# PetoAdam/RayZen

Measured on AMD Instinct MI355X. Metric: Msamples/s (rays x spp / s) at 1080p, higher is better.
Workload: dtype f32; 1 GPU; configs[1]: bunny stand-in (bunny69312, 69324 tris incl. floor) 1920x1080, 64 spp per frame (64 spp-equivalents of work per GPU), 4 bounces, 2 lights; width=1920, height=1080, spp_per_gpu=64, spp_total=64, bounces=4, triangles=69324, floor=cube scaled (8, 0.5, 8) at y = -3 (main.cpp:378), parallelism=tiles8x8-roundrobin-x1

## Files before the change

### include/rayzen_hip.h

```cpp
#ifndef RAYZEN_HIP_H
#define RAYZEN_HIP_H

#include <stddef.h>
#include <stdint.h>

#ifdef __cplusplus
extern "C" {
#endif


typedef struct rz_triangle {
    float v0[3]; float pad0;
    float v1[3]; float pad1;
    float v2[3]; float pad2;
    int32_t materialIndex;
    int32_t tail_pad[3];
} rz_triangle;

typedef struct rz_bvh_node {
    float boundsMin[3]; int32_t leftFirst;
    float boundsMax[3]; int32_t count;
} rz_bvh_node;

typedef struct rz_bvh_instance {
// ... 152 lines not shown
int rz_rebuild_geometry(rz_ctx* ctx, double max_ratio, rz_mesh_quality* out, size_t cap, size_t* n_meshes, unsigned flags );

int rz_read_binding(rz_ctx* ctx, rz_binding binding, void* out, size_t bytes, size_t* needed);

int rz_set_frame(rz_ctx* ctx, const rz_frame_params* params);

int rz_set_stream(rz_ctx* ctx, void* hip_stream);
int rz_bind_accum(rz_ctx* ctx, void* device_rgba, size_t bytes);

int rz_render(rz_ctx* ctx);
int rz_render_counted(rz_ctx* ctx, rz_counters* out);
int rz_sync(rz_ctx* ctx);

int rz_clear_accum(rz_ctx* ctx);

int rz_read_accum(rz_ctx* ctx, float* rgba, size_t bytes);

int rz_resolve_rgba8(rz_ctx* ctx, uint8_t* rgba8, size_t bytes);

typedef struct rz_present_params {
    float   fps;
    int32_t show_fps;
    int32_t show_lights;
    int32_t show_bvh;
    int32_t bvh_mode;
    int32_t selected_blas;
    int32_t selected_tri;
} rz_present_params;
int rz_present(rz_ctx* ctx, const rz_present_params* params, uint8_t* rgba8, size_t rgba8_bytes, float* rgb32f,
               size_t rgb32f_bytes);

int rz_last_render_ms(rz_ctx* ctx, float* ms, int* launches);
int rz_render_history_ms(rz_ctx* ctx, float* ms, int cap);
const char* rz_last_kernel_name(const rz_ctx* ctx);

void* rz_accum_device_ptr(rz_ctx* ctx);

int rz_debug_fail_alloc(rz_ctx* ctx, int nth);

void* rz_stream_handle(rz_ctx* ctx);

typedef struct rz_group rz_group;
#define RZ_GROUP_ID_BYTES 128
#define RZ_GROUP_LOOPBACK 0x10000u
int       rz_group_rccl_version(int* version);
int       rz_group_unique_id(void* id128);
rz_group* rz_group_create(int ndev, const int* devices, unsigned flags);
rz_group* rz_group_create_rank(int device, int rank, int nranks, const void* id128, unsigned flags);
void      rz_group_destroy(rz_group* g);
const char* rz_group_last_error(const rz_group* g);
int       rz_group_size(const rz_group* g);
const char* rz_group_transport(const rz_group* g);
int       rz_group_set_transport(rz_group* g, const char* name);
int       rz_group_local_count(const rz_group* g);
int       rz_group_rank(const rz_group* g, int local);
rz_ctx*   rz_group_ctx(rz_group* g, int local);
int rz_group_upload(rz_group* g, rz_binding binding, const void* data, size_t bytes);
int rz_group_update(rz_group* g, rz_binding binding, size_t offset, const void* data, size_t bytes);
int rz_group_set_frame(rz_group* g, const rz_frame_params* params);
int rz_group_render(rz_group* g);
int rz_group_reduce(rz_group* g, int root);
int rz_group_sync(rz_group* g);
int rz_group_last_reduce_ms(rz_group* g, float* root_ms, float* max_ms);
int rz_group_read_frame(rz_group* g, float* rgba, size_t bytes);
void* rz_group_frame_device_ptr(rz_group* g);

int rz_debug_poke_backstop(rz_ctx* ctx, unsigned bits);

int rz_debug_read_layout(rz_ctx* ctx, int which, void* out, size_t bytes, size_t* needed);

typedef struct rz_launch_plan {
    int64_t groups;
    int64_t grid;
    int32_t per_claim;
    int32_t claim_units;
    int32_t batches_per_pixel;
    int32_t pixels_per_wave;
    int32_t lds_stack_entries;
    int32_t overflow_entries;
    int32_t transparent;
    int32_t scratch_mib;
} rz_launch_plan;
int rz_debug_last_plan(rz_ctx* ctx, rz_launch_plan* out);

typedef struct rz_ray {
    float    origin[3];
    float    max_dist;
    float    dir[3];
    uint32_t reserved;
} rz_ray;
typedef struct rz_hit {
    float   t;
    float   point[3];
    float   normal[3];
    int32_t material, instance, triangle, prim, reserved;
} rz_hit;
typedef struct rz_visibility {
    float   visibility;
    int32_t lit;
} rz_visibility;
#define RZ_RAYS_HOST        1u
#define RZ_RAYS_INCOHERENT  2u
int rz_trace_rays(rz_ctx* ctx, const rz_ray* rays, rz_hit* hits, size_t n, unsigned flags);
int rz_shadow_rays(rz_ctx* ctx, const rz_ray* rays, rz_visibility* out, size_t n, unsigned flags);

typedef struct rz_editor_params {
    float ambient[3];  float pad0;
    float clear[4];
} rz_editor_params;
#define RZ_EDITOR_HOST       1u
#define RZ_EDITOR_INCOHERENT 2u
int rz_render_editor(rz_ctx* ctx, const rz_frame_params* frame, const rz_editor_params* params,
                     uint8_t* rgba8, size_t rgba8_bytes, float* rgb32f, size_t rgb32f_bytes,
                     rz_hit* hits, size_t hits_bytes, unsigned flags);

typedef struct rz_denoise_params {
    int32_t iterations;
    float   sigma_color, sigma_normal, sigma_plane;
    int32_t demodulate;
    int32_t reserved[3];
} rz_denoise_params;
#define RZ_DENOISE_HOST 1u
int rz_denoise(rz_ctx* ctx, const rz_denoise_params* params, const float* rgba_in, size_t rgba_in_bytes,
               float* rgb32f, size_t rgb32f_bytes, rz_hit* guides, size_t guides_bytes, unsigned flags);
int rz_present_denoised(rz_ctx* ctx, const rz_present_params* present, const rz_denoise_params* params,
                        uint8_t* rgba8, size_t rgba8_bytes, float* rgb32f, size_t rgb32f_bytes);

typedef struct rz_temporal_params {
    float   alpha, alpha_moments;
    int32_t max_history;
    float   normal_cos, plane_tol;
    int32_t iterations;
    float   sigma_l, sigma_normal, sigma_plane;
    int32_t demodulate;
    int32_t reserved[6];
} rz_temporal_params;
#define RZ_TEMPORAL_HOST 1u
#define RZ_TEMPORAL_KEEP 4u
int rz_denoise_temporal(rz_ctx* ctx, const rz_temporal_params* params, const float* rgba_in, size_t rgba_in_bytes,
                        float* rgb32f, size_t rgb32f_bytes, rz_hit* guides, size_t guides_bytes,
                        float* stats, size_t stats_bytes, unsigned flags);
int rz_present_temporal(rz_ctx* ctx, const rz_present_params* present, const rz_temporal_params* params,
                        uint8_t* rgba8, size_t rgba8_bytes, float* rgb32f, size_t rgb32f_bytes);
int rz_temporal_reset(rz_ctx* ctx);
int rz_debug_read_temporal(rz_ctx* ctx, int which, void* out, size_t bytes, size_t* needed);

typedef struct rz_display_params {
    int32_t exposure_mode;
    float   exposure;
    float   key;
    float   min_exposure, max_exposure;
    float   adapt;
    int32_t low_permille, high_permille;
    int32_t curve;
    float   white;
    int32_t transfer;
    int32_t reserved[5];
} rz_display_params;

typedef struct rz_display_info {
    float    exposure;
    float    target;
    float    log2_mean;
    uint32_t counted, below, above;
    uint32_t histogram[128];
} rz_display_info;
// ... 130 lines not shown
```

### rayzen_amd/_lib.py

```python
import ctypes as C
import os

import numpy as np

_HERE = os.path.dirname(os.path.abspath(__file__))
HIP_SO = os.environ.get("RAYZEN_HIP_SO") or os.path.join(_HERE, "lib", "librayzen_hip.so")
HOST_SO = os.path.join(_HERE, "lib", "librayzen_host.so")

HIP_SYMBOLS = (
    "rz_create", "rz_destroy", "rz_last_error", "rz_upload", "rz_update", "rz_update_transforms", "rz_build_blas", "rz_build_geometry", "rz_read_binding",
    "rz_set_frame", "rz_set_stream",
    "rz_bind_accum", "rz_render", "rz_render_counted", "rz_sync", "rz_clear_accum", "rz_read_accum",
    "rz_resolve_rgba8", "rz_present", "rz_last_render_ms", "rz_render_history_ms", "rz_last_kernel_name", "rz_accum_device_ptr", "rz_version", "rz_sizeof",
    "rz_debug_fail_alloc", "rz_debug_read_layout", "rz_debug_last_plan", "rz_source_hash", "rz_stream_handle", "rz_device_count",
    "rz_group_rccl_version", "rz_group_unique_id", "rz_group_create", "rz_group_create_rank", "rz_group_destroy",
    "rz_group_last_error", "rz_group_size", "rz_group_local_count", "rz_group_rank", "rz_group_ctx", "rz_group_upload",
    "rz_group_update", "rz_group_set_frame", "rz_group_render", "rz_group_reduce", "rz_group_sync", "rz_group_read_frame",
    "rz_group_frame_device_ptr", "rz_group_last_reduce_ms", "rz_group_transport", "rz_group_set_transport", "rz_abi_version", "rz_debug_poke_backstop", "rz_math_flavour",
    "rz_trace_rays", "rz_shadow_rays", "rz_render_editor", "rz_denoise", "rz_present_denoised", "rz_refit_geometry",
    "rz_denoise_temporal", "rz_present_temporal", "rz_temporal_reset", "rz_debug_read_temporal",
    "rz_display", "rz_present_display", "rz_display_reset", "rz_display_state",
    "rz_skin_create", "rz_skin_pose", "rz_skin_destroy", "rz_skin_last_kernel_ms",
    "rz_geometry_quality", "rz_rebuild_geometry",
    "rz_upscale", "rz_present_upscaled", "rz_upscale_seethrough", "rz_present_upscaled_seethrough",
    "rz_antialias", "rz_present_antialiased", "rz_antialias_seethrough", "rz_present_antialiased_seethrough",
    "rz_render_cost", "rz_cost_view", "rz_present_cost",
    "rz_coverage", "rz_outline",
)
ABI_VERSION = 5
HOST_SYMBOLS = (
    "rzh_load_obj", "rzh_build_blas", "rzh_build_tlas", "rzh_world_bounds", "rzh_scene_create",
    "rzh_scene_destroy", "rzh_scene_add_mesh", "rzh_scene_add_object", "rzh_scene_set_transform",
    "rzh_scene_build", "rzh_scene_set_blas_builder", "rzh_scene_update_dynamic", "rzh_scene_buffer", "rzh_scene_depths",
    "rzh_scene_save_cache", "rzh_scene_load_cache", "rzh_scene_build_cached",
    "rzh_camera_matrices", "rzh_mat_translate", "rzh_mat_scale", "rzh_mat_rotate", "rzh_mat_inverse",
    "rzh_make_cube", "rzh_make_blob", "rzh_version", "rzh_refit_blas", "rzh_scene_refit_mesh", "rzh_skin_triangles",
    "rzh_blas_sah_cost", "rzh_scene_rebuild_mesh",
)


class FrameParams(C.Structure):
    _fields_ = [("width", C.c_int32), ("height", C.c_int32),
                ("inv_view", C.c_float * 16), ("inv_proj", C.c_float * 16),
                ("view", C.c_float * 16), ("proj", C.c_float * 16),
                ("cam_pos", C.c_float * 3),
                ("num_lights", C.c_int32), ("bounce_budget", C.c_int32),
                ("spp", C.c_int32), ("sample_base", C.c_int32),
                ("tile_rank", C.c_int32), ("tile_nranks", C.c_int32)]


COUNTER_FIELDS = ("samples", "traversals", "tlas_nodes", "tlas_leaf_indices", "instances",
                  "blas_nodes", "triangles", "materials", "light_fetches", "pixels",
                  "scatters", "diffuse_scatters", "hemi_draws", "lit_lights", "triangles_past_u")


class PresentParams(C.Structure):
    _fields_ = [("fps", C.c_float), ("show_fps", C.c_int32), ("show_lights", C.c_int32), ("show_bvh", C.c_int32),
                ("bvh_mode", C.c_int32), ("selected_blas", C.c_int32), ("selected_tri", C.c_int32)]


class BvhNode(C.Structure):
    _fields_ = [("boundsMin", C.c_float * 3), ("leftFirst", C.c_int32), ("boundsMax", C.c_float * 3), ("count", C.c_int32)]


class MeshBuild(C.Structure):
    _fields_ = [("first_triangle", C.c_size_t), ("n_triangles", C.c_size_t), ("node_offset", C.c_int32),
                ("index_offset", C.c_int32), ("n_nodes", C.c_int32), ("depth", C.c_int32), ("root", BvhNode)]


class LaunchPlan(C.Structure):
    _fields_ = [("groups", C.c_int64), ("grid", C.c_int64), ("per_claim", C.c_int32), ("claim_units", C.c_int32),
                ("batches_per_pixel", C.c_int32), ("pixels_per_wave", C.c_int32), ("lds_stack_entries", C.c_int32),
                ("overflow_entries", C.c_int32), ("transparent", C.c_int32), ("scratch_mib", C.c_int32)]


class Ray(C.Structure):
    _fields_ = [("origin", C.c_float * 3), ("max_dist", C.c_float), ("dir", C.c_float * 3), ("reserved", C.c_uint32)]


class Hit(C.Structure):
    _fields_ = [("t", C.c_float), ("point", C.c_float * 3), ("normal", C.c_float * 3), ("material", C.c_int32),
                ("instance", C.c_int32), ("triangle", C.c_int32), ("prim", C.c_int32), ("reserved", C.c_int32)]


class Visibility(C.Structure):
    _fields_ = [("visibility", C.c_float), ("lit", C.c_int32)]


RAYS_HOST, RAYS_INCOHERENT = 1, 2


class EditorParams(C.Structure):
    _fields_ = [("ambient", C.c_float * 3), ("pad0", C.c_float), ("clear", C.c_float * 4)]


EDITOR_HOST, EDITOR_INCOHERENT = 1, 2


class DenoiseParams(C.Structure):
    _fields_ = [("iterations", C.c_int32), ("sigma_color", C.c_float), ("sigma_normal", C.c_float), ("sigma_plane", C.c_float),
                ("demodulate", C.c_int32), ("reserved", C.c_int32 * 3)]


DENOISE_HOST = 1


class TemporalParams(C.Structure):
    _fields_ = [("alpha", C.c_float), ("alpha_moments", C.c_float), ("max_history", C.c_int32), ("normal_cos", C.c_float),
                ("plane_tol", C.c_float), ("iterations", C.c_int32), ("sigma_l", C.c_float), ("sigma_normal", C.c_float),
                ("sigma_plane", C.c_float), ("demodulate", C.c_int32), ("reserved", C.c_int32 * 6)]
# ... 145 lines not shown
        L.rz_destroy.restype, L.rz_destroy.argtypes = None, [vp]
        L.rz_last_error.restype, L.rz_last_error.argtypes = C.c_char_p, [vp]
        L.rz_upload.restype, L.rz_upload.argtypes = i, [vp, i, vp, sz]
        L.rz_update.restype, L.rz_update.argtypes = i, [vp, i, sz, vp, sz]
        L.rz_update_transforms.restype, L.rz_update_transforms.argtypes = i, [vp, vp, sz]
        L.rz_read_binding.restype, L.rz_read_binding.argtypes = i, [vp, i, vp, sz, C.POINTER(sz)]
        L.rz_build_blas.restype, L.rz_build_blas.argtypes = i, [vp, vp, sz, vp, sz, vp, C.POINTER(sz), C.POINTER(C.c_int), C.POINTER(C.c_float)]
        L.rz_build_geometry.restype, L.rz_build_geometry.argtypes = i, [vp, vp, sz, C.POINTER(MeshBuild), sz]
        L.rz_set_frame.restype, L.rz_set_frame.argtypes = i, [vp, C.POINTER(FrameParams)]
        L.rz_set_stream.restype, L.rz_set_stream.argtypes = i, [vp, vp]
        L.rz_bind_accum.restype, L.rz_bind_accum.argtypes = i, [vp, vp, sz]
        L.rz_render.restype, L.rz_render.argtypes = i, [vp]
        L.rz_render_counted.restype, L.rz_render_counted.argtypes = i, [vp, C.POINTER(Counters)]
        L.rz_sync.restype, L.rz_sync.argtypes = i, [vp]
        L.rz_clear_accum.restype, L.rz_clear_accum.argtypes = i, [vp]
        L.rz_read_accum.restype, L.rz_read_accum.argtypes = i, [vp, vp, sz]
        L.rz_resolve_rgba8.restype, L.rz_resolve_rgba8.argtypes = i, [vp, vp, sz]
        L.rz_present.restype, L.rz_present.argtypes = i, [vp, C.POINTER(PresentParams), vp, sz, vp, sz]
        L.rz_last_render_ms.restype, L.rz_last_render_ms.argtypes = i, [vp, C.POINTER(C.c_float), C.POINTER(i)]
        L.rz_render_history_ms.restype, L.rz_render_history_ms.argtypes = i, [vp, C.POINTER(C.c_float), i]
        L.rz_last_kernel_name.restype, L.rz_last_kernel_name.argtypes = C.c_char_p, [vp]
        L.rz_accum_device_ptr.restype, L.rz_accum_device_ptr.argtypes = vp, [vp]
        L.rz_version.restype, L.rz_version.argtypes = C.c_char_p, []
        L.rz_sizeof.restype, L.rz_sizeof.argtypes = sz, [i]
        L.rz_debug_fail_alloc.restype, L.rz_debug_fail_alloc.argtypes = i, [vp, i]
        L.rz_debug_read_layout.restype, L.rz_debug_read_layout.argtypes = i, [vp, i, vp, sz, C.POINTER(sz)]
        L.rz_debug_last_plan.restype, L.rz_debug_last_plan.argtypes = i, [vp, C.POINTER(LaunchPlan)]
        L.rz_source_hash.restype, L.rz_source_hash.argtypes = C.c_char_p, []
        L.rz_stream_handle.restype, L.rz_stream_handle.argtypes = vp, [vp]
        L.rz_device_count.restype, L.rz_device_count.argtypes = i, []
        L.rz_group_rccl_version.restype, L.rz_group_rccl_version.argtypes = i, [C.POINTER(i)]
        L.rz_group_unique_id.restype, L.rz_group_unique_id.argtypes = i, [vp]
        L.rz_group_create.restype, L.rz_group_create.argtypes = vp, [i, C.POINTER(i), C.c_uint]
        L.rz_group_create_rank.restype, L.rz_group_create_rank.argtypes = vp, [i, i, i, vp, C.c_uint]
        L.rz_group_destroy.restype, L.rz_group_destroy.argtypes = None, [vp]
        L.rz_group_last_error.restype, L.rz_group_last_error.argtypes = C.c_char_p, [vp]
        L.rz_group_size.restype, L.rz_group_size.argtypes = i, [vp]
        L.rz_group_local_count.restype, L.rz_group_local_count.argtypes = i, [vp]
        L.rz_group_rank.restype, L.rz_group_rank.argtypes = i, [vp, i]
        L.rz_group_ctx.restype, L.rz_group_ctx.argtypes = vp, [vp, i]
        L.rz_group_upload.restype, L.rz_group_upload.argtypes = i, [vp, i, vp, sz]
        L.rz_group_update.restype, L.rz_group_update.argtypes = i, [vp, i, sz, vp, sz]
        L.rz_group_set_frame.restype, L.rz_group_set_frame.argtypes = i, [vp, C.POINTER(FrameParams)]
        L.rz_group_render.restype, L.rz_group_render.argtypes = i, [vp]
        L.rz_group_reduce.restype, L.rz_group_reduce.argtypes = i, [vp, i]
        L.rz_group_sync.restype, L.rz_group_sync.argtypes = i, [vp]
        L.rz_group_read_frame.restype, L.rz_group_read_frame.argtypes = i, [vp, vp, sz]
        L.rz_group_frame_device_ptr.restype, L.rz_group_frame_device_ptr.argtypes = vp, [vp]
        for name, res, args in (("rz_group_last_reduce_ms", i, [vp, C.POINTER(C.c_float), C.POINTER(C.c_float)]),
                                ("rz_group_transport", C.c_char_p, [vp]),
                                ("rz_group_set_transport", i, [vp, C.c_char_p]),
                                ("rz_abi_version", i, []), ("rz_debug_poke_backstop", i, [vp, C.c_uint]), ("rz_math_flavour", i, []),
                                ("rz_trace_rays", i, [vp, vp, vp, sz, C.c_uint]), ("rz_shadow_rays", i, [vp, vp, vp, sz, C.c_uint]),
                                ("rz_render_editor", i, [vp, C.POINTER(FrameParams), vp, vp, sz, vp, sz, vp, sz, C.c_uint]),
                                ("rz_denoise", i, [vp, vp, vp, sz, vp, sz, vp, sz, C.c_uint]),
                                ("rz_present_denoised", i, [vp, C.POINTER(PresentParams), vp, vp, sz, vp, sz]),
                                ("rz_refit_geometry", i, [vp, vp, sz, sz, C.c_uint]),
                                ("rz_denoise_temporal", i, [vp, vp, vp, sz, vp, sz, vp, sz, vp, sz, C.c_uint]),
                                ("rz_present_temporal", i, [vp, C.POINTER(PresentParams), vp, vp, sz, vp, sz]),
                                ("rz_temporal_reset", i, [vp]),
                                ("rz_debug_read_temporal", i, [vp, i, vp, sz, C.POINTER(sz)]),
                                ("rz_display", i, [vp, vp, vp, sz, vp, sz, vp, sz, C.c_uint]),
                                ("rz_present_display", i, [vp, C.POINTER(PresentParams), vp, i, vp, vp, sz, vp, sz]),
                                ("rz_display_reset", i, [vp]),
                                ("rz_display_state", i, [vp, C.POINTER(DisplayInfo)]),
                                ("rz_skin_create", i, [vp, sz, sz, vp, vp, i, vp, i, C.POINTER(i)]),
                                ("rz_skin_pose", i, [vp, i, vp, vp, C.c_uint]),
                                ("rz_skin_destroy", i, [vp, i]),
                                ("rz_skin_last_kernel_ms", i, [vp, C.POINTER(C.c_float)]),
                                ("rz_geometry_quality", i, [vp, vp, sz, C.POINTER(sz)]),
                                ("rz_rebuild_geometry", i, [vp, C.c_double, vp, sz, C.POINTER(sz), C.c_uint]),
                                ("rz_upscale", i, [vp, vp, vp, sz, vp, sz, vp, sz, C.c_uint]),
                                ("rz_present_upscaled", i, [vp, C.POINTER(PresentParams), vp, vp, i, vp, vp, sz, vp, sz]),
                                ("rz_upscale_seethrough", i, [vp, vp, vp, vp, sz, vp, sz, vp, sz, vp, sz, C.c_uint]),
                                ("rz_present_upscaled_seethrough", i, [vp, C.POINTER(PresentParams), vp, vp, vp, i, vp, vp, sz, vp, sz]),
                                ("rz_antialias", i, [vp, vp, vp, sz, vp, sz, vp, sz, vp, sz, C.c_uint]),
                                ("rz_present_antialiased", i, [vp, C.POINTER(PresentParams), vp, vp, i, vp, vp, sz, vp, sz]),
                                ("rz_antialias_seethrough", i, [vp, vp, vp, vp, sz, vp, sz, vp, sz, vp, sz, vp, sz, C.c_uint]),
                                ("rz_present_antialiased_seethrough", i, [vp, C.POINTER(PresentParams), vp, vp, vp, i, vp, vp, sz, vp, sz]),
                                ("rz_render_cost", i, [vp, vp, vp, sz, C.POINTER(Counters), C.c_uint]),
                                ("rz_cost_view", i, [vp, vp, vp, sz, vp, sz, vp, C.c_uint]),
                                ("rz_present_cost", i, [vp, C.POINTER(PresentParams), vp, vp, sz, vp, sz]),
                                ("rz_coverage", i, [vp, C.POINTER(FrameParams), vp, vp, sz, vp, sz, C.c_uint]),
                                ("rz_outline", i, [vp, vp, vp, sz, vp, sz, vp, sz, vp, sz, C.c_uint])):
            try:
                fn = getattr(L, name)
                fn.restype, fn.argtypes = res, args
            except AttributeError:
                if not os.environ.get("RAYZEN_HIP_SO"):
                    raise
        if hasattr(L, "rz_abi_version") and L.rz_abi_version() != ABI_VERSION and not os.environ.get("RAYZEN_HIP_SO"):
            raise RuntimeError(f"{HIP_SO} speaks ABI revision {L.rz_abi_version()}, this binding {ABI_VERSION}: rebuild (python -m rayzen_amd.build)")
        _hip = L
    return _hip


def host():
    global _host
    if _host is None:
        if not os.path.exists(HOST_SO):
            raise RuntimeError(f"{HOST_SO} is missing: run `python -m rayzen_amd.build`")
        L = C.CDLL(HOST_SO)
        vp, i, sz, f = C.c_void_p, C.c_int, C.c_size_t, C.c_float
        L.rzh_load_obj.restype, L.rzh_load_obj.argtypes = i, [C.c_char_p, i, vp, i]
        L.rzh_build_blas.restype, L.rzh_build_blas.argtypes = i, [vp, i, vp, vp, C.POINTER(i)]
        L.rzh_build_tlas.restype, L.rzh_build_tlas.argtypes = i, [vp, i, vp, vp, C.POINTER(i)]
        L.rzh_refit_blas.restype, L.rzh_refit_blas.argtypes = i, [vp, i, vp, i, vp]
        L.rzh_scene_refit_mesh.restype, L.rzh_scene_refit_mesh.argtypes = i, [vp, i, vp, i]
        L.rzh_blas_sah_cost.restype, L.rzh_blas_sah_cost.argtypes = C.c_double, [vp, i]
        L.rzh_scene_rebuild_mesh.restype, L.rzh_scene_rebuild_mesh.argtypes = i, [vp, i]
        L.rzh_skin_triangles.restype, L.rzh_skin_triangles.argtypes = i, [vp, vp, i, vp, i, vp, vp, i, vp]
        L.rzh_world_bounds.restype, L.rzh_world_bounds.argtypes = None, [vp, vp, vp, vp]
        L.rzh_scene_create.restype, L.rzh_scene_create.argtypes = vp, []
        L.rzh_scene_destroy.restype, L.rzh_scene_destroy.argtypes = None, [vp]
        L.rzh_scene_add_mesh.restype, L.rzh_scene_add_mesh.argtypes = i, [vp, vp, i]
        L.rzh_scene_add_object.restype, L.rzh_scene_add_object.argtypes = i, [vp, i, vp]
        L.rzh_scene_set_transform.restype, L.rzh_scene_set_transform.argtypes = i, [vp, i, vp]
        L.rzh_scene_build.restype, L.rzh_scene_build.argtypes = i, [vp, i]
        L.rzh_scene_set_blas_builder.restype, L.rzh_scene_set_blas_builder.argtypes = i, [vp, vp, vp]
        L.rzh_scene_update_dynamic.restype, L.rzh_scene_update_dynamic.argtypes = i, [vp]
        L.rzh_scene_buffer.restype, L.rzh_scene_buffer.argtypes = vp, [vp, i, C.POINTER(sz)]
        L.rzh_scene_save_cache.restype, L.rzh_scene_save_cache.argtypes = i, [vp, C.c_char_p]
        L.rzh_scene_load_cache.restype, L.rzh_scene_load_cache.argtypes = i, [vp, C.c_char_p]
        L.rzh_scene_build_cached.restype, L.rzh_scene_build_cached.argtypes = i, [vp, C.c_char_p, i, C.POINTER(i * 5)]
        L.rzh_scene_depths.restype, L.rzh_scene_depths.argtypes = None, [vp, C.POINTER(i), C.POINTER(i)]
        L.rzh_camera_matrices.restype = None
        L.rzh_camera_matrices.argtypes = [vp, vp, vp, f, f, f, f, vp, vp, vp, vp]
        for n in ("rzh_mat_translate", "rzh_mat_scale"):
            getattr(L, n).restype, getattr(L, n).argtypes = None, [vp, vp, vp]
        L.rzh_mat_rotate.restype, L.rzh_mat_rotate.argtypes = None, [vp, f, vp, vp]
        L.rzh_mat_inverse.restype, L.rzh_mat_inverse.argtypes = None, [vp, vp]
        L.rzh_make_cube.restype, L.rzh_make_cube.argtypes = i, [i, vp, i]
        L.rzh_make_blob.restype, L.rzh_make_blob.argtypes = i, [i, f, C.c_uint, i, vp, i]
        L.rzh_version.restype, L.rzh_version.argtypes = C.c_char_p, []
        _host = L
    return _host
```

### rayzen_amd/csrc/hip/rz_context.hip

```cpp
#include <hip/hip_runtime.h>

#include <algorithm>
#include <cmath>
#include <cstdarg>
#include <cstdio>
#include <cstdlib>
#include <cstring>
#include <map>
#include <new>
#include <string>
#include <tuple>
#include <limits>
#include <vector>

#include "rayzen_hip.h"
#include "rz_internal.h"
#include "rz_device_math.h"


using namespace rz;

namespace {

thread_local std::string g_last_error = "";
// ... 21 lines not shown
struct RefitView {
    std::tuple<int, int, int> key;
    int rankBase = 0;
    std::vector<int> levelStart;
    int maxNode = 0;
};

struct SkinRig {
    size_t first = 0, n = 0;
    int nBones = 0, nMorphs = 0;
    DevBuf dRest, dSkin, dMorphs;
    void release() { dRest.release(); dSkin.release(); dMorphs.release(); }
};

constexpr int kNumBindings = 10;
size_t elem_size(int b) {
    switch (b) {
        case RZ_BIND_TRIANGLES: return sizeof(rz_triangle);
        case RZ_BIND_MATERIALS: return sizeof(rz_material);
        case RZ_BIND_LIGHTS: return sizeof(rz_light);
        case RZ_BIND_TLAS_NODES: return sizeof(rz_bvh_node);
        case RZ_BIND_TLAS_INDICES: return sizeof(int32_t);
        case RZ_BIND_BLAS_NODES: return sizeof(rz_bvh_node);
        case RZ_BIND_BLAS_INDICES: return sizeof(int32_t);
        case RZ_BIND_INSTANCES: return sizeof(rz_bvh_instance);
        default: return 0;
    }
}
int group_of(int b) {
    switch (b) {
        case RZ_BIND_TRIANGLES: return kTris;
        case RZ_BIND_BLAS_NODES: case RZ_BIND_BLAS_INDICES: return kBlas;
        case RZ_BIND_INSTANCES: case RZ_BIND_TLAS_NODES: case RZ_BIND_TLAS_INDICES: return kTlas;
        default: return kNoGroup;
    }
}

}

struct rz_ctx {
    int device = 0;
    unsigned flags = 0;
    hipStream_t ownStream = nullptr;
    hipStream_t stream = nullptr;
    static constexpr int kRing = 64;
    hipEvent_t evStart[kRing] = {}, evStop[kRing] = {};
    int ringHead = 0;
    int ringCount = 0;
    bool timed = false;
    int lastLaunches = 0;
    float hemi0[3] = {0.0f, 0.0f, 0.0f};
    long long triNValid = -1;
    long long lastGrid = 0;
    rz_launch_plan lastPlan{};
    bool lastCompact = false;
    bool lastGlobalPool = false;
    std::string err;

    std::vector<unsigned char> host[kNumBindings];
    bool present[kNumBindings] = {};
    Residency where[kNumGroups];
    bool geomDirty = true, instDirty = true, tlasDirty = true, matDirty = true, lightDirty = true;

    DevBuf dPairs, dTris, dInst, dTlasNodes, dTlasIdx, dMat, dLight, dCounters, dResolve, dGroupCtr, dBlasOvf;
    std::map<std::tuple<int, int, int>, BlasView> views;
    std::vector<DevPair> hPairs;
    std::vector<DevTri> hTris;
    int maxBlasDepth = 1, tlasDepth = 1;

    bool haveFrame = false;
    rz_frame_params frame{};
    DevBuf ownAccum, dIor;
    DevBuf dXforms, dInstRef, dTlasScratch, dProjBoxes, dBuildWs, dTlasDfs, dTriN;
    int nTlasDfs = 0;
    int* tlasHostCounts = nullptr;
    int devTlasNodes = 0;
    bool sceneHasTransparency = true;
    const char* lastKernel = "";
    void* extAccum = nullptr;
    size_t extAccumBytes = 0;
    int failAllocCountdown = 0;
    DevBuf dRawNodes, dRawIdx, dRawTris, dRelayoutWs, dClaimScratch;
    DevBuf dSnap;
    DevBuf dWavePools, dWaitMeta;
    size_t lastScratchBytes = 0;
    int* relayoutPinned = nullptr;
    bool layoutOnDevice = false;
    long long devPairsUsed = 0, devTrisUsed = 0;
    bool matChangedSinceLayout = false;
    unsigned devTransparent = 0;
    bool irregularBoxes = false;
    size_t devNodes = 0, devIdx = 0;
    std::map<int, rz_bvh_node> devRoots;
    DevBuf dRayOvf, dRayIn, dRayOut, dRayInstOff;
    bool rayInstOffStale = true;
    DevBuf dDnGuide, dDnPing, dDnPong, dDnOut;
    DevBuf dTmpCol[2], dTmpMom[2], dTmpHits[2], dTmpInst[2], dTmpSame;
    int tmpCur = 0;
    bool tmpValid = false;
    int tmpW = 0, tmpH = 0;
    size_t tmpInst = 0;
    float tmpView[16] = {}, tmpProj[16] = {}, tmpInvProj[16] = {}, tmpCam[3] = {};
    DevBuf dDisplay;
    DevBuf dUpGuideLo, dUpGuideHi, dUpOut;
    DevBuf dStGuideLo, dStGuideHi;
    DevBuf dAasList, dAasCounts;
    unsigned long long layoutGen = 0;
    unsigned long long refitGen = ~0ull;
    std::vector<RefitView> refitViews;
    DevBuf dRefitRank, dRefitInstView, dRefitViewOff, dRefitFlags, dRefitRoots;
    unsigned char* refitPinned = nullptr;
    size_t refitPinnedCap = 0;
    std::map<int, SkinRig> rigs;
    int nextRig = 0;
    DevBuf dSkinOut, dSkinBones, dSkinWeights;
    hipEvent_t evSkin[2] = {nullptr, nullptr};
    bool skinTimed = false;
    DevBuf dQualViews, dQualPartials, dQualCost;
    int qualBlocks = 0;
    std::map<std::tuple<int, int, int>, double> costBuilt;
    unsigned long long costGen = ~0ull;
    DevBuf dCost, dCostCounters, dCostPartials, dCostStats, dCostOut;
    bool costValid = false;
    int costW = 0, costH = 0, costSpp = 0;
    DevBuf dCovSets;
    long long covSets = 0;
    size_t covStride = 0, covCount = 0;
};

namespace {

int fail(rz_ctx* c, int code, const char* fmt, ...) {
    char buf[512];
    va_list ap;
    va_start(ap, fmt);
    vsnprintf(buf, sizeof buf, fmt, ap);
    va_end(ap);
    try {
        if (c) c->err = buf;
        g_last_error = buf;
    } catch (...) { }
    return code;
}

template <class F>
int guarded(rz_ctx* c, const char* what, F&& body) {
    try {
        if (c) {
            const hipError_t e = hipSetDevice(c->device);
            if (e != hipSuccess) return fail(c, RZ_ERR_HIP, "%s: hipSetDevice(%d): %s", what, c->device, hipGetErrorString(e));
        }
        return body();
    } catch (const std::bad_alloc&) {
        return fail(c, RZ_ERR_NO_MEMORY, "%s: out of host memory", what);
    } catch (const std::exception& e) {
        return fail(c, RZ_ERR_HIP, "%s: %s", what, e.what());
    } catch (...) {
        return fail(c, RZ_ERR_HIP, "%s: unknown C++ exception", what);
    }
}
void alloc_point(rz_ctx* c) {
    if (c->failAllocCountdown > 0 && --c->failAllocCountdown == 0) throw std::bad_alloc();
}

#define RZ_HIP(c, call)                                                                            \
    do {                                                                                           \
// ... 579 lines not shown
    int place() { return host && total ? ensure(c, c->dRayOut, total) : RZ_OK; }
    template <class T>
    T* dev(int slot) const {
        if (!host || !out[slot].ptr) return static_cast<T*>(out[slot].ptr);
        return reinterpret_cast<T*>(static_cast<char*>(c->dRayOut.p) + out[slot].off);
    }
    int fetch() {
        const char* base = static_cast<const char*>(c->dRayOut.p);
        for (int k = 0; k < n; ++k)
            if (out[k].ptr) RZ_HIP(c, hipMemcpyAsync(out[k].ptr, base + out[k].off, out[k].bytes, hipMemcpyDeviceToHost, c->stream));
        RZ_HIP(c, hipStreamSynchronize(c->stream));
        return RZ_OK;
    }
};

int render_samples(rz_ctx* c, KParams K, bool counted, int evSlot) {
    K.nSlots = K.nLocalTiles * 64;
    int rc = ensure_group_counter(c);
    if (rc != RZ_OK) return rc;
    K.groupCounter = static_cast<unsigned*>(c->dGroupCtr.p);
    const SamplesPlan plan = plan_render_samples(K.spp, K.nSlots, c->sceneHasTransparency);
#ifndef RZ_GLASS_WAVES_PER_CU
#define RZ_GLASS_WAVES_PER_CU 16
#endif
#ifndef RZ_OPAQUE_WAVES_PER_CU
#define RZ_OPAQUE_WAVES_PER_CU 16
#endif
    rc = size_blas_stack(c, K, samples_lds_extra(c->sceneHasTransparency, plan.compact) + (size_t)K.tlasStackCap * 256,
                         c->sceneHasTransparency ? RZ_GLASS_WAVES_PER_CU : RZ_OPAQUE_WAVES_PER_CU,
                         plan.perClaim > 0 ? plan.grid : 0, c->dBlasOvf);
    if (rc != RZ_OK) return rc;
    K.wslots = nullptr; K.wslotStride = 0; K.slotFloats = 0; K.nWaitSlots = 0; K.wmeta = nullptr; K.drainEachClaim = 0; K.claimUnits = 0; K.claimScratchFloats = 0;
    K.wpool = nullptr; K.wpoolStride = 0; K.wpoolChunk = 0;
    if (plan.compact && K.maxBounces < 32768) {
        long long chunk = RZ_WPOOL_CHUNK;
        if (const char* e = std::getenv("RZ_WPOOL_CHUNK")) chunk = std::max<long long>(1, std::atoll(e));
        const int nBatches = (K.spp + 63) / 64;
        const int groupsPerClaim = std::max(1, plan.perClaim);
        int nSlots = std::max(2 * groupsPerClaim, 16 / nBatches);
        if (const char* e = std::getenv("RZ_WAIT_SLOTS")) nSlots = std::max(2 * groupsPerClaim, std::atoi(e));
        nSlots = std::min(nSlots, 64);
        const size_t stride = (size_t)chunk + (size_t)plan.claimUnits * 64 + 64 + (c->sceneHasTransparency ? (size_t)RZ_GLATE_CAP : 0);
        const size_t slotFloats = (size_t)nBatches * 384 + (c->sceneHasTransparency ? 64 : 0);
        const size_t claimScratchFloats = (size_t)groupsPerClaim * slotFloats;
        bool snapOn = true;
        if (const char* e = std::getenv("RZ_GLASS_SNAPSHOT")) snapOn = std::atoi(e) != 0;
        size_t slotPad = 0;
        if (const char* e = std::getenv("RZ_SLOT_STRIDE_PAD")) slotPad = (size_t)std::max(0, std::atoi(e));
        const char* forceNo = std::getenv("RZ_DEBUG_NO_POOL_MEMORY");
        if (nSlots >= groupsPerClaim && !(forceNo && std::atoi(forceNo) != 0) && (!c->sceneHasTransparency || snapOn) &&
            ensure_optional(c->dWavePools, (size_t)plan.grid * stride * RZ_GPOOL_FIELDS * sizeof(unsigned)) &&
            ensure_optional(c->dClaimScratch, (size_t)plan.grid * (claimScratchFloats + nSlots * slotFloats + slotPad) * sizeof(float)) &&
            ensure_optional(c->dWaitMeta, (size_t)plan.grid * 4 * nSlots * sizeof(int32_t))) {
            K.wpool = static_cast<unsigned*>(c->dWavePools.p);
            K.wpoolStride = (uint32_t)stride;
            K.wpoolChunk = (uint32_t)chunk;
            K.wslots = static_cast<float*>(c->dClaimScratch.p);
            K.wslotStride = (uint32_t)(claimScratchFloats + nSlots * slotFloats + slotPad);
            K.claimUnits = plan.claimUnits;
            K.claimScratchFloats = (uint32_t)claimScratchFloats;
            K.glassBoxHint = 1;
            if (const char* e = std::getenv("RZ_GLASS_BOX_HINT")) K.glassBoxHint = std::atoi(e) != 0 ? 1 : 0;
            K.slotFloats = (uint32_t)slotFloats;
            K.nWaitSlots = nSlots;
            K.wmeta = static_cast<int32_t*>(c->dWaitMeta.p);
            K.drainEachClaim = plan.drainEachClaim ? 1 : 0;
        }
    }
    c->lastGlobalPool = K.wpool != nullptr && K.drainEachClaim == 0;
    c->lastCompact = K.wpool != nullptr;
    c->lastScratchBytes = K.wpool ? (size_t)plan.grid * ((size_t)K.wpoolStride * RZ_GPOOL_FIELDS * 4 + (size_t)K.wslotStride * 4 + (size_t)16 * K.nWaitSlots) : 0;
    K.snap = nullptr; K.snapStride = 0;
    if (c->sceneHasTransparency && plan.perClaim > 0) {
        bool on = true;
        if (const char* e = std::getenv("RZ_GLASS_SNAPSHOT")) on = std::atoi(e) != 0;
        const size_t stride = (size_t)(RZ_SNAP_FIELDS + RZ_SNAP_TALLY + RZ_GVER_ROWS) * 64 + (size_t)RZ_GLATE_FIELDS * RZ_GLATE_CAP;
        if (on) {
            rc = ensure(c, c->dSnap, (size_t)plan.grid * stride * sizeof(float));
            if (rc != RZ_OK) return rc;
            K.snap = static_cast<float*>(c->dSnap.p);
            K.snapStride = (uint32_t)stride;
        }
    }
    RZ_HIP(c, hipEventRecord(c->evStart[evSlot], c->stream));
    if (K.nSlots > 0) launch_render_samples(K, counted, c->sceneHasTransparency, c->stream);
    RZ_HIP(c, hipEventRecord(c->evStop[evSlot], c->stream));
    c->lastLaunches = K.nSlots > 0 ? 1 : 0;
    c->lastGrid = plan.grid;
    c->lastPlan = rz_launch_plan{plan.groups, plan.grid, plan.perClaim, (plan.compact && K.wpool) ? plan.claimUnits : 0,
                                 (K.spp + 63) / 64, K.spp >= 64 ? 1 : 64 / K.spp, K.blasStackCap, K.blasOvfCap,
                                 c->sceneHasTransparency ? 1 : 0, (int32_t)((c->lastScratchBytes + (1u << 20) - 1) >> 20)};
    return RZ_OK;
}

int frame_kparams(rz_ctx* c, KParams& K, int spp, int sampleBase) {
    const rz_frame_params& f = c->frame;
    scene_kparams(c, K);
    K.nLights = std::max(0, std::min<int>(f.num_lights, (int)hostCount<rz_light>(c, RZ_BIND_LIGHTS)));
    K.width = f.width; K.height = f.height;
    K.tilesX = (f.width + RZ_TILE_W - 1) / RZ_TILE_W;
    K.tilesY = (f.height + RZ_TILE_H - 1) / RZ_TILE_H;
    const int nTiles = K.tilesX * K.tilesY;
    K.tileRank = f.tile_rank; K.tileNRanks = f.tile_nranks;
    K.nLocalTiles = (nTiles - f.tile_rank + f.tile_nranks - 1) / f.tile_nranks;
    K.maxBounces = f.bounce_budget > 0 ? f.bounce_budget : 5;
    K.spp = spp; K.sampleBase = sampleBase;
    std::memcpy(K.invView, f.inv_view, 64);
    std::memcpy(K.invProj, f.inv_proj, 64);
    std::memcpy(K.camPos, f.cam_pos, 12);
    std::memcpy(K.hemi0, c->hemi0, 12);
    {
        const long long nIdx = tlas_index_count(c);
        long long minInst = RZ_SPREAD_MIN_INSTANCES;
        if (const char* e = std::getenv("RZ_SPREAD_MIN_INSTANCES")) minInst = std::atoll(e);
        K.spreadTrace = (minInst > 0 && nIdx >= minInst) ? 1 : 0;
    }
    const size_t perWave = (size_t)K.blasStackCap * 512 + (size_t)K.tlasStackCap * 256 + 4864;
    if (perWave * 4 > 160 * 1024)
        return fail(c, RZ_ERR_BAD_SCENE, "BLAS depth %d needs %zu B of LDS stack per wave; the limit is %d", c->maxBlasDepth, perWave, 40 * 1024);
    return RZ_OK;
}

int do_render(rz_ctx* c, bool counted, rz_counters* out) {
    if (!c) return fail(nullptr, RZ_ERR_INVALID_ARG, "null context");
    if (!c->haveFrame) return fail(c, RZ_ERR_NOT_READY, "rz_set_frame has not been called");
    RZ_HIP(c, hipSetDevice(c->device));
    int rc = finalize(c);
    if (rc != RZ_OK) return rc;
    const rz_frame_params& f = c->frame;
    const size_t nPix = (size_t)f.width * f.height;
    float4* accum = nullptr;
    if (c->extAccum) {
        if (c->extAccumBytes < nPix * 16) return fail(c, RZ_ERR_BUFFER_SIZE, "bound accumulation buffer holds %zu bytes, frame needs %zu", c->extAccumBytes, nPix * 16);
        accum = static_cast<float4*>(c->extAccum);
    } else {
        accum = static_cast<float4*>(c->ownAccum.p);
    }
    KParams K{};
    K.accum = accum;
    K.ior = static_cast<float*>(c->dIor.p);
    rc = frame_kparams(c, K, f.spp, f.sample_base);
    if (rc != RZ_OK) return rc;
    if (counted) {
        rc = ensure(c, c->dCounters, sizeof(DevCounters) + 160 * sizeof(unsigned long long));
        if (rc != RZ_OK) return rc;
        RZ_HIP(c, hipMemsetAsync(c->dCounters.p, 0, sizeof(DevCounters) + 160 * sizeof(unsigned long long), c->stream));
        K.counters = static_cast<DevCounters*>(c->dCounters.p);
    }
    const int slot = c->ringHead;
    if (use_samples(c)) {
        rc = render_samples(c, K, counted, slot);
        if (rc != RZ_OK) return rc;
        c->lastKernel = c->sceneHasTransparency ? (c->lastCompact ? "rz_render_samples<glass>+pool" : "rz_render_samples<glass>")
                                                : (c->lastGlobalPool ? "rz_render_samples+pool" : "rz_render_samples");
    } else {
        RZ_HIP(c, hipEventRecord(c->evStart[slot], c->stream));
        launch_render_pixels(K, counted, c->stream);
        RZ_HIP(c, hipEventRecord(c->evStop[slot], c->stream));
        c->lastLaunches = 1;
        c->lastKernel = "rz_render_pixels";
        c->lastPlan = rz_launch_plan{K.nLocalTiles, K.nLocalTiles, 0, 0, (K.spp + 63) / 64, 64, K.blasStackCap, 0, c->sceneHasTransparency ? 1 : 0, 0};
    }
    RZ_HIP(c, hipGetLastError());
    c->ringHead = (slot + 1) % rz_ctx::kRing;
    c->ringCount = std::min(c->ringCount + 1, (int)rz_ctx::kRing);
    c->timed = true;
    if (counted && out) {
        DevCounters h{};
        RZ_HIP(c, hipMemcpyAsync(&h, c->dCounters.p, sizeof h, hipMemcpyDeviceToHost, c->stream));
        RZ_HIP(c, hipStreamSynchronize(c->stream));
// ... 41 lines not shown
#define RZ_SOURCE_HASH "unstamped"
#endif
static const char rz_stamp[] = "RZSRCHASH:" RZ_SOURCE_HASH;
const char* rz_source_hash(void) { return rz_stamp + 10; }
const char* rz_version(void) { return "rayzen_hip 0.5 (gfx950)"; }
int rz_abi_version(void) { return RZ_ABI_VERSION; }
int rz_math_flavour(void) { return RZ_MATH_FLAVOUR; }

int rz_device_count(void) {
    int n = 0;
    return hipGetDeviceCount(&n) == hipSuccess && n > 0 ? n : 0;
}

size_t rz_sizeof(int which) {
    switch (which) {
        case 0: return sizeof(rz_triangle);
        case 1: return sizeof(rz_bvh_node);
        case 2: return sizeof(rz_bvh_instance);
        case 3: return sizeof(rz_material);
        case 4: return sizeof(rz_light);
        case 5: return sizeof(rz_frame_params);
        case 6: return sizeof(rz_counters);
        case 7: return sizeof(rz_ray);
        case 8: return sizeof(rz_hit);
        case 9: return sizeof(rz_visibility);
        case 10: return sizeof(rz_editor_params);
        case 11: return sizeof(rz_denoise_params);
        case 12: return sizeof(rz_temporal_params);
        case 14: return sizeof(rz_display_params);
        case 15: return sizeof(rz_display_info);
        case 17: return sizeof(rz_skin_triangle);
        case 18: return sizeof(rz_morph_triangle);
        case 20: return sizeof(rz_mesh_quality);
        case 21: return sizeof(rz_upscale_params);
        case 23: return sizeof(rz_seethrough_params);
        case 24: return sizeof(rz_chain);
        case 26: return sizeof(rz_antialias_params);
        case 28: return sizeof(rz_pixel_cost);
        case 29: return sizeof(rz_cost_params);
        case 30: return sizeof(rz_cost_view_params);
        case 31: return sizeof(rz_cost_stats);
        case 33: return sizeof(rz_coverage_params);
        case 34: return sizeof(rz_instance_coverage);
        case 35: return sizeof(rz_outline_params);
        default: return 0;
    }
}

const char* rz_last_error(const rz_ctx* ctx) { return ctx ? ctx->err.c_str() : g_last_error.c_str(); }

rz_ctx* rz_create(int device, unsigned flags) {
    int n = 0;
    hipError_t e = hipGetDeviceCount(&n);
    if (e != hipSuccess || n <= 0) { fail(nullptr, RZ_ERR_NO_DEVICE, "no HIP device (%s)", hipGetErrorString(e)); return nullptr; }
    if (device < 0 || device >= n) { fail(nullptr, RZ_ERR_INVALID_ARG, "device %d of %d", device, n); return nullptr; }
    rz_ctx* c = new (std::nothrow) rz_ctx();
    if (!c) { fail(nullptr, RZ_ERR_HIP, "out of host memory"); return nullptr; }
    c->device = device;
    c->flags = flags;
    bool ok = hipSetDevice(device) == hipSuccess &&
              hipStreamCreateWithFlags(&c->ownStream, hipStreamNonBlocking) == hipSuccess;
    for (int i = 0; ok && i < rz_ctx::kRing; ++i)
        ok = hipEventCreate(&c->evStart[i]) == hipSuccess && hipEventCreate(&c->evStop[i]) == hipSuccess;
    if (!ok) {
        fail(nullptr, RZ_ERR_HIP, "cannot create stream/events on device %d", device);
        rz_destroy(c);
        return nullptr;
    }
    c->stream = c->ownStream;
    const int hrc = compute_hemi0(c->hemi0, c->stream);
    if (hrc != 0) {
        fail(nullptr, RZ_ERR_HIP, "cannot run the set-up kernel on device %d: %s", device, hipGetErrorString((hipError_t)(-hrc)));
        rz_destroy(c);
        return nullptr;
    }
    return c;
}

void rz_destroy(rz_ctx* c) {
    if (!c) return;
    (void)hipSetDevice(c->device);
    if (c->stream) (void)hipStreamSynchronize(c->stream);
    for (DevBuf* b : {&c->dPairs, &c->dTris, &c->dInst, &c->dTlasNodes, &c->dTlasIdx, &c->dMat, &c->dLight,
                      &c->dCounters, &c->dResolve, &c->dGroupCtr, &c->dBlasOvf, &c->ownAccum, &c->dIor, &c->dXforms, &c->dInstRef, &c->dTlasScratch, &c->dProjBoxes, &c->dBuildWs, &c->dTlasDfs, &c->dTriN, &c->dRawNodes, &c->dRawIdx, &c->dRawTris, &c->dRelayoutWs, &c->dClaimScratch, &c->dWavePools, &c->dWaitMeta, &c->dSnap,
                      &c->dRayOvf, &c->dRayIn, &c->dRayOut, &c->dRayInstOff, &c->dDnGuide, &c->dDnPing, &c->dDnPong, &c->dDnOut,
                      &c->dRefitRank, &c->dRefitInstView, &c->dRefitViewOff, &c->dRefitFlags, &c->dRefitRoots,
                      &c->dTmpCol[0], &c->dTmpCol[1], &c->dTmpMom[0], &c->dTmpMom[1], &c->dTmpHits[0], &c->dTmpHits[1],
                      &c->dTmpInst[0], &c->dTmpInst[1], &c->dTmpSame, &c->dDisplay, &c->dSkinOut, &c->dSkinBones, &c->dSkinWeights,
                      &c->dQualViews, &c->dQualPartials, &c->dQualCost, &c->dUpGuideLo, &c->dUpGuideHi, &c->dUpOut,
                      &c->dStGuideLo, &c->dStGuideHi, &c->dAasList, &c->dAasCounts,
                      &c->dCost, &c->dCostCounters, &c->dCostPartials, &c->dCostStats, &c->dCostOut, &c->dCovSets})
        b->release();
    for (auto& kv : c->rigs) kv.second.release();
    for (hipEvent_t e : c->evSkin) if (e) (void)hipEventDestroy(e);
    if (c->refitPinned) (void)hipHostFree(c->refitPinned);
    if (c->tlasHostCounts) (void)hipHostFree(c->tlasHostCounts);
    if (c->relayoutPinned) (void)hipHostFree(c->relayoutPinned);
    for (int i = 0; i < rz_ctx::kRing; ++i) {
        if (c->evStart[i]) (void)hipEventDestroy(c->evStart[i]);
        if (c->evStop[i]) (void)hipEventDestroy(c->evStop[i]);
    }
    if (c->ownStream) (void)hipStreamDestroy(c->ownStream);
    delete c;
}

static int host_copy_for(rz_ctx* c, int binding, bool replacing = false) {
    const int g = group_of(binding);
    return g == kNoGroup ? RZ_OK : need_host(c, g, replacing ? binding : -1);
}
static void mark_dirty(rz_ctx* c, int binding) {
    switch (binding) {
        case RZ_BIND_MATERIALS: c->matDirty = true; break;
        case RZ_BIND_LIGHTS: c->lightDirty = true; break;
        case RZ_BIND_TLAS_NODES: case RZ_BIND_TLAS_INDICES: c->tlasDirty = true; break;
        case RZ_BIND_INSTANCES: c->instDirty = true; break;
        default: c->geomDirty = true; break;
    }
}
static int host_copy_changed(rz_ctx* c, int binding) {
    const int g = group_of(binding);
    if (g != kNoGroup) { const int rc = host_changed(c, g); if (rc != RZ_OK) return rc; }
    if (g == kBlas) drop_built_costs(c);
    mark_dirty(c, binding);
    return RZ_OK;
}

static int upload_impl(rz_ctx* c, rz_binding binding, const void* data, size_t bytes) {
    if (!c) return fail(nullptr, RZ_ERR_INVALID_ARG, "null context");
    const size_t es = elem_size((int)binding);
    if (es == 0) return fail(c, RZ_ERR_INVALID_ARG, "unknown binding %d", (int)binding);
    if (bytes % es) return fail(c, RZ_ERR_INVALID_ARG, "binding %d: %zu bytes is not a multiple of the %zu-byte element", (int)binding, bytes, es);
    if (bytes && !data) return fail(c, RZ_ERR_INVALID_ARG, "null data");
    alloc_point(c);
    c->host[binding].reserve(bytes);
    { const int rc = host_copy_for(c, binding, true); if (rc != RZ_OK) return rc; }
    c->host[binding].assign(static_cast<const unsigned char*>(data), static_cast<const unsigned char*>(data) + bytes);
    if (binding == RZ_BIND_TRIANGLES || binding == RZ_BIND_BLAS_NODES || binding == RZ_BIND_BLAS_INDICES || binding == RZ_BIND_INSTANCES)
        c->tmpValid = false;
    c->present[binding] = true;
    return host_copy_changed(c, binding);
}

static int update_impl(rz_ctx* c, rz_binding binding, size_t offset, const void* data, size_t bytes) {
    if (!c) return fail(nullptr, RZ_ERR_INVALID_ARG, "null context");
    if (elem_size((int)binding) == 0) return fail(c, RZ_ERR_INVALID_ARG, "unknown binding %d", (int)binding);
    if (!c->present[binding]) return fail(c, RZ_ERR_NOT_READY, "binding %d has not been uploaded", (int)binding);
    if (bytes && !data) return fail(c, RZ_ERR_INVALID_ARG, "null data");
    { const int rc = host_copy_for(c, binding); if (rc != RZ_OK) return rc; }
    if (offset > c->host[binding].size() || bytes > c->host[binding].size() - offset)
        return fail(c, RZ_ERR_OUT_OF_RANGE, "binding %d: update [%zu,+%zu) past its %zu bytes", (int)binding, offset, bytes, c->host[binding].size());
    if (bytes == 0) return RZ_OK;
    if (std::memcmp(c->host[binding].data() + offset, data, bytes) == 0) return RZ_OK;
    std::memcpy(c->host[binding].data() + offset, data, bytes);
    return host_copy_changed(c, binding);
}

static int tlas_rebuild(rz_ctx* c, const float* transforms, size_t n);

static int update_transforms_impl(rz_ctx* c, const float* transforms, size_t n) {
    if (!c) return fail(nullptr, RZ_ERR_INVALID_ARG, "null context");
    if (!transforms && n) return fail(c, RZ_ERR_INVALID_ARG, "null transforms");
    RZ_HIP(c, hipSetDevice(c->device));
    int rc = finalize(c);
    if (rc != RZ_OK) return rc;
    const size_t nInst = hostCount<rz_bvh_instance>(c, RZ_BIND_INSTANCES);
    if (n != nInst) return fail(c, RZ_ERR_INVALID_ARG, "%zu transforms for %zu instances", n, nInst);
    return tlas_rebuild(c, transforms, n);
// ... 2659 lines not shown
        return antialias_impl(c, params, rgb_in, rgb_in_bytes, rgb32f, rgb32f_bytes, guides, guides_bytes, edges, edges_bytes, flags);
    });
}
int rz_present_antialiased(rz_ctx* c, const rz_present_params* present, const rz_antialias_params* antialias,
                           const rz_display_params* display, int source, const void* filter_params, uint8_t* rgba8, size_t rgba8_bytes,
                           float* rgb32f, size_t rgb32f_bytes) {
    return guarded(c, "rz_present_antialiased", [&] {
        return present_antialiased_impl(c, present, antialias, display, source, filter_params, rgba8, rgba8_bytes, rgb32f, rgb32f_bytes);
    });
}
int rz_antialias_seethrough(rz_ctx* c, const rz_antialias_params* params, const rz_seethrough_params* seethrough, const float* rgb_in,
                            size_t rgb_in_bytes, float* rgb32f, size_t rgb32f_bytes, rz_hit* guides, size_t guides_bytes, rz_chain* chains,
                            size_t chains_bytes, uint8_t* edges, size_t edges_bytes, unsigned flags) {
    return guarded(c, "rz_antialias_seethrough", [&] {
        return antialias_impl(c, params, rgb_in, rgb_in_bytes, rgb32f, rgb32f_bytes, guides, guides_bytes, edges, edges_bytes, flags,
                              seethrough ? seethrough : &kSeethroughDefaults, chains, chains_bytes);
    });
}
int rz_present_antialiased_seethrough(rz_ctx* c, const rz_present_params* present, const rz_antialias_params* antialias,
                                      const rz_seethrough_params* seethrough, const rz_display_params* display, int source,
                                      const void* filter_params, uint8_t* rgba8, size_t rgba8_bytes, float* rgb32f, size_t rgb32f_bytes) {
    return guarded(c, "rz_present_antialiased_seethrough", [&] {
        return present_antialiased_impl(c, present, antialias, display, source, filter_params, rgba8, rgba8_bytes, rgb32f, rgb32f_bytes,
                                        seethrough ? seethrough : &kSeethroughDefaults);
    });
}
int rz_render_cost(rz_ctx* c, const rz_cost_params* params, rz_pixel_cost* cost, size_t cost_bytes, rz_counters* totals, unsigned flags) {
    return guarded(c, "rz_render_cost", [&] { return render_cost_impl(c, params, cost, cost_bytes, totals, flags); });
}
int rz_cost_view(rz_ctx* c, const rz_cost_view_params* params, const rz_pixel_cost* cost, size_t cost_bytes, float* rgb32f,
                 size_t rgb32f_bytes, rz_cost_stats* stats, unsigned flags) {
    return guarded(c, "rz_cost_view", [&] { return cost_view_impl(c, params, cost, cost_bytes, rgb32f, rgb32f_bytes, stats, flags); });
}
int rz_present_cost(rz_ctx* c, const rz_present_params* present, const rz_cost_view_params* params, uint8_t* rgba8, size_t rgba8_bytes,
                    float* rgb32f, size_t rgb32f_bytes) {
    return guarded(c, "rz_present_cost", [&] { return present_cost_impl(c, present, params, rgba8, rgba8_bytes, rgb32f, rgb32f_bytes); });
}
int rz_coverage(rz_ctx* c, const rz_frame_params* frame, const rz_coverage_params* params, rz_instance_coverage* coverage,
                size_t coverage_bytes, int32_t* ids, size_t ids_bytes, unsigned flags) {
    return guarded(c, "rz_coverage", [&] { return coverage_impl(c, frame, params, coverage, coverage_bytes, ids, ids_bytes, flags); });
}
int rz_outline(rz_ctx* c, const rz_outline_params* params, const int32_t* ids, size_t ids_bytes, const uint32_t* selected,
               size_t n_instances, uint8_t* rgba8, size_t rgba8_bytes, float* rgb32f, size_t rgb32f_bytes, unsigned flags) {
    return guarded(c, "rz_outline", [&] {
        return outline_impl(c, params, ids, ids_bytes, selected, n_instances, rgba8, rgba8_bytes, rgb32f, rgb32f_bytes, flags);
    });
}
int rz_display_reset(rz_ctx* c) {
    return guarded(c, "rz_display_reset", [&] { return display_reset_impl(c); });
}
int rz_display_state(rz_ctx* c, rz_display_info* out) {
    return guarded(c, "rz_display_state", [&] { return display_state_impl(c, out); });
}
int rz_debug_read_layout(rz_ctx* c, int which, void* out, size_t bytes, size_t* needed) {
    return guarded(c, "rz_debug_read_layout", [&]() -> int {
        if (!c) return fail(nullptr, RZ_ERR_INVALID_ARG, "null context");
        if (which < 0 || which > 2) return fail(c, RZ_ERR_INVALID_ARG, "which = %d", which);
        RZ_HIP(c, hipSetDevice(c->device));
        int rc = finalize(c);
        if (rc != RZ_OK) return rc;
        size_t have;
        const void* src;
        if (which == 0) { have = (c->layoutOnDevice ? (size_t)c->devPairsUsed : c->hPairs.size()) * sizeof(DevPair); src = c->dPairs.p; }
        else if (which == 1) { have = (c->layoutOnDevice ? (size_t)c->devTrisUsed : c->hTris.size()) * sizeof(DevTri); src = c->dTris.p; }
        else { have = (size_t)c->nTlasDfs * sizeof(TlasDfs); src = c->dTlasDfs.p; }
        if (needed) *needed = have;
        if (!out) return RZ_OK;
        if (bytes < have) return fail(c, RZ_ERR_BUFFER_SIZE, "layout %d holds %zu bytes, buffer has %zu", which, have, bytes);
        if (have) {
            RZ_HIP(c, hipMemcpyAsync(out, src, have, hipMemcpyDeviceToHost, c->stream));
            RZ_HIP(c, hipStreamSynchronize(c->stream));
        }
        return RZ_OK;
    });
}

int rz_debug_last_plan(rz_ctx* c, rz_launch_plan* out) {
    if (!c || !out) return fail(c, RZ_ERR_INVALID_ARG, "rz_debug_last_plan: null argument");
    if (!c->timed) return fail(c, RZ_ERR_NOT_READY, "rz_debug_last_plan: nothing has been rendered yet");
    *out = c->lastPlan;
    return RZ_OK;
}

int rz_debug_fail_alloc(rz_ctx* c, int nth) {
    if (!c) return fail(nullptr, RZ_ERR_INVALID_ARG, "null context");
    c->failAllocCountdown = nth > 0 ? nth : 0;
    return RZ_OK;
}

}
```

### rayzen_amd/csrc/hip/rz_internal.h

```cpp
#pragma once
#include <hip/hip_runtime.h>

#include "rayzen_hip.h"
#include "rz_scene_dev.h"

namespace rz {

template <class C>
__device__ __forceinline__ void store_colour(float4* dst, float* rgb, size_t p, const C& c, float w) {
    if (dst) dst[p] = make_float4(c.x, c.y, c.z, w);
    if (rgb) {
        rgb[3 * p] = c.x;
        rgb[3 * p + 1] = c.y;
        rgb[3 * p + 2] = c.z;
    }
}

#ifndef RZ_WAVES_PER_BLOCK
#define RZ_WAVES_PER_BLOCK 1
#endif
constexpr int WAVES_PER_BLOCK = RZ_WAVES_PER_BLOCK;
#ifndef RZ_MIN_WAVES_PER_SIMD
#define RZ_MIN_WAVES_PER_SIMD 2
#endif
void launch_render_pixels(const KParams& K, bool counted, hipStream_t stream);
SamplesPlan plan_render_samples(int spp, int nSlots, bool glass);
size_t samples_lds_extra(bool glass, bool compact);
void launch_render_samples(const KParams& K, bool counted, bool glass, hipStream_t stream);
void launch_resolve(const float4* accum, uchar4* out, int n, hipStream_t stream);
int compute_hemi0(float out[3], hipStream_t stream);
#ifdef RZ_PROF
void dump_wave_log(int nWaves);
#endif
#ifdef RZ_GSTATS
void dump_gstats();
#endif

constexpr int RZ_RAYS_WAVES_PER_CU = 16;
struct RaysLaunch {
    const void* rays;
    void* out;
    int n;
    long long grid;
    bool shadow, spread;
    const int32_t* instTriOff;
    unsigned* errWord;
};
long long rays_grid(long long n);
void launch_rays(const KParams& K, const RaysLaunch& R, hipStream_t stream);

struct EditorLaunch {
    float view[16], proj[16];
    float ambient[3];
    float clear[4];
    long long units;
    int unitsX;
    int rows;
    long long grid;
    bool spread;
    uchar4* rgba8;
    float* rgb32f;
    float4* hits;
    const int32_t* instTriOff;
    unsigned* errWord;
};
void launch_editor(const KParams& K, const EditorLaunch& E, hipStream_t stream);

struct DenoiseGuideLaunch {
    long long units;
    int unitsX;
    long long grid;
    float4* guide;
    float4* hits;
    const int32_t* instTriOff;
    unsigned* errWord;
};
void launch_denoise_guides(const KParams& K, const DenoiseGuideLaunch& G, hipStream_t stream);
struct DenoiseLaunch {
    const float4* accum;
    const float4* src;
    const float4* guide;
    const DevMaterial* materials;
    float4* dst;
    float* rgb;
    int width, height;
    int step;
    float invColor;
    float sigmaNormal;
    float planeScale;
    int demodulate;
};
void launch_denoise_pass(const DenoiseLaunch& D, bool first, bool last, hipStream_t stream);
void launch_denoise_resolve(const DenoiseLaunch& D, hipStream_t stream);

struct UpscaleLaunch {
    const float* in3;
    const float4* in4;
    const float4* guideLo;
    const float4* guideHi;
    const DevMaterial* materials;
    float4* dst;
    float* rgb;
    int w, h;
    int s;
    float sigmaNormal;
    float planeScale;
    int demodulate;
};
void launch_upscale_gather(const UpscaleLaunch& U, hipStream_t stream);

constexpr int RZ_AA_QUEUE = 128;
// ... 266 lines not shown
```

### rayzen_amd/csrc/hip/rz_kernels.hip

```cpp
#include <hip/hip_runtime.h>

#include <algorithm>
#include <cstdlib>
#include <cstdio>
#include <vector>

#include "rayzen_hip.h"
#include "rz_path.h"
#include "rz_internal.h"

namespace rz {


#ifdef RZ_PROF
__device__ unsigned long long rz_wave_log[1 << 17][3];
#endif
#ifdef RZ_GSTATS
__device__ unsigned long long rz_gstats[8];
#define RZ_GSTAT(i, n) do { if ((threadIdx.x & 63) == 0) atomicAdd(&rz_gstats[i], (unsigned long long)(n)); } while (0)
#else
#define RZ_GSTAT(i, n) do { } while (0)
#endif

template <bool COUNT>
__global__ __launch_bounds__(WAVES_PER_BLOCK * 64, RZ_MIN_WAVES_PER_SIMD) void rz_render_pixels(const KParams K) {
#ifdef RZ_PROF
    const unsigned long long wl_t0 = __builtin_amdgcn_s_memrealtime();
#endif
    extern __shared__ __attribute__((aligned(16))) unsigned char lds_raw[];
    const int lane = threadIdx.x & 63;
    const int wave = threadIdx.x >> 6;
    const size_t perWave = (size_t)K.blasStackCap * 64 * sizeof(uint2) + (size_t)K.tlasStackCap * 64 * sizeof(int);
    unsigned char* base = lds_raw + perWave * wave;
    const BlasStackT<false> bstk{reinterpret_cast<uint2*>(base) + lane, nullptr, K.blasStackCap};

    const int localTile = blockIdx.x * WAVES_PER_BLOCK + wave;
    if (localTile >= K.nLocalTiles) return;
    const int tile = localTile * K.tileNRanks + K.tileRank;
    const int tx = tile % K.tilesX, ty = tile / K.tilesX;
    const int px = tx * RZ_TILE_W + (lane & 7), py = ty * RZ_TILE_H + (lane >> 3);
    const bool inside = px < K.width && py < K.height;
    const size_t pix = (size_t)py * K.width + px;

    Tally c = {};
    Path P;
    P.mode = MODE_DONE;
    P.samp = K.sampleBase;
    P.sampEnd = inside ? K.sampleBase + K.spp : K.sampleBase;
    float alpha = 0.0f;
    if (inside) {
        const float fragx = (float)px + 0.5f, fragy = (float)py + 0.5f;
        P.uv.x = fragx / (float)K.width;
        P.uv.y = fragy / (float)K.height;
        P.fragSum = fragx + fragy;
        if (K.sampleBase == 0) {
            P.color = mk3(0.0f, 0.0f, 0.0f);
            P.ior = 1.0f;
        } else {
            const float4 a = K.accum[pix];
            P.color = mk3(a.x, a.y, a.z);
            alpha = a.w;
            P.ior = K.ior[pix];
        }
    }
#ifdef RZ_PROF
    unsigned long long tTrace = 0, tAdv = 0, tBegin = 0;
#endif
    while (P.samp < P.sampEnd) {
#ifdef RZ_PROF
        RZ_SITE(c, 6);
        unsigned long long t0 = __builtin_amdgcn_s_memtime();
        if (P.mode == MODE_DONE) { RZ_SITE(c, 7); begin_sample<COUNT>(K, P, c); }
        unsigned long long t1 = __builtin_amdgcn_s_memtime();
        HitRec h;
        const bool found = trace_closest<COUNT, false>(K, P.o, P.d, h, bstk, c);
        unsigned long long t2 = __builtin_amdgcn_s_memtime();
        advance<COUNT>(K, P, found, h, c);
        unsigned long long t3 = __builtin_amdgcn_s_memtime();
        tBegin += t1 - t0; tTrace += t2 - t1; tAdv += t3 - t2;
#else
        if (P.mode == MODE_DONE) begin_sample<COUNT>(K, P, c);
        HitRec h;
        const bool found = trace_closest<COUNT, false>(K, P.o, P.d, h, bstk, c);
        advance<COUNT>(K, P, found, h, c);
#endif
    }
#ifdef RZ_PROF
    if (lane == 0 && localTile < (1 << 17)) {
        rz_wave_log[localTile][0] = wl_t0;
        rz_wave_log[localTile][1] = __builtin_amdgcn_s_memrealtime();
        rz_wave_log[localTile][2] = (unsigned long long)__builtin_amdgcn_s_getreg((3 << 0) | (0 << 6) | (31 << 11)) |
                                    ((unsigned long long)__builtin_amdgcn_s_getreg((20 << 0) | (0 << 6) | (31 << 11)) << 32);
    }
    if (COUNT) {
        unsigned long long* pr = reinterpret_cast<unsigned long long*>(K.counters + 1);
        for (int k = 0; k < 16; ++k) atomicAdd(&pr[k], (unsigned long long)c.p[k]);
        if (lane == 0) { atomicAdd(&pr[16], tBegin); atomicAdd(&pr[17], tTrace); atomicAdd(&pr[18], tAdv); }
    }
#endif
    if (inside) {
        K.accum[pix] = make_float4(P.color.x, P.color.y, P.color.z, alpha + (float)K.spp);
        K.ior[pix] = P.ior;
    }
    if (COUNT) {
        DevCounters* g = K.counters;
        atomicAdd(&g->samples, (unsigned long long)c.samples);
        atomicAdd(&g->traversals, (unsigned long long)c.traversals);
        atomicAdd(&g->tlas_nodes, (unsigned long long)c.tlas_nodes);
        atomicAdd(&g->tlas_leaf_indices, (unsigned long long)c.tlas_leaf_indices);
        atomicAdd(&g->instances, (unsigned long long)c.instances);
        atomicAdd(&g->blas_nodes, (unsigned long long)c.blas_nodes);
        atomicAdd(&g->triangles, (unsigned long long)c.triangles);
        atomicAdd(&g->materials, (unsigned long long)c.materials);
        atomicAdd(&g->light_fetches, (unsigned long long)c.light_fetches);
        atomicAdd(&g->scatters, (unsigned long long)c.scatters);
        atomicAdd(&g->diffuse_scatters, (unsigned long long)c.diffuse_scatters);
        atomicAdd(&g->hemi_draws, (unsigned long long)c.hemi_draws);
        atomicAdd(&g->lit_lights, (unsigned long long)c.lit_lights);
        atomicAdd(&g->triangles_past_u, (unsigned long long)c.triangles_past_u);
        if (inside) atomicAdd(&g->pixels, 1ull);
    }
}

#ifndef RZ_SAMPLES_MIN_WAVES
#define RZ_SAMPLES_MIN_WAVES 4
#endif
#ifndef RZ_SAMPLES_MIN_WAVES_GLASS
#define RZ_SAMPLES_MIN_WAVES_GLASS 4
#endif
__device__ __forceinline__ int slot_x(int l, bool morton) { return morton ? ((l & 1) | ((l >> 1) & 2) | ((l >> 2) & 4)) : (l & 7); }
__device__ __forceinline__ int slot_y(int l, bool morton) { return morton ? (((l >> 1) & 1) | ((l >> 2) & 2) | ((l >> 3) & 4)) : (l >> 3); }
#ifdef RZ_PROF
__device__ __forceinline__ void rz_prof_rounds(const Tally& c, unsigned long long* pr) {
    for (int k = 0; k < 8; ++k) {
        unsigned x = c.ps[k];
        for (int o = 32; o > 0; o >>= 1) x += __shfl_xor(x, o);
        if ((threadIdx.x & 63) == 0 && x) atomicAdd(&pr[132 + k], (unsigned long long)x);
    }
    for (int r = 0; r < 8; ++r) {
        for (int k = 0; k < 10; ++k) {
            unsigned x = c.rp[r][k];
            for (int o = 32; o > 0; o >>= 1) x += __shfl_xor(x, o);
            if ((threadIdx.x & 63) == 0 && x) atomicAdd(&pr[32 + 11 * r + k], (unsigned long long)x);
        }
        if ((threadIdx.x & 63) == 0 && c.rt[r]) atomicAdd(&pr[32 + 11 * r + 10], c.rt[r]);
    }
    for (int k = 0; k < 18; ++k) {
        unsigned x = c.sx[k / 6][k % 6];
        for (int o = 32; o > 0; o >>= 1) x += __shfl_xor(x, o);
        if ((threadIdx.x & 63) == 0 && x) atomicAdd(&pr[140 + k], (unsigned long long)x);
    }
}
#endif
__device__ __forceinline__ void tally_add(Tally& a, const Tally& b) {
    a.traversals += b.traversals; a.tlas_nodes += b.tlas_nodes; a.tlas_leaf_indices += b.tlas_leaf_indices;
    a.instances += b.instances; a.blas_nodes += b.blas_nodes; a.triangles += b.triangles; a.materials += b.materials;
    a.light_fetches += b.light_fetches; a.samples += b.samples;
    a.triangles_past_u += b.triangles_past_u; a.scatters += b.scatters; a.diffuse_scatters += b.diffuse_scatters; a.hemi_draws += b.hemi_draws; a.lit_lights += b.lit_lights;
#ifdef RZ_PROF
    for (int k = 0; k < 16; ++k) a.p[k] += b.p[k];
    for (int k = 0; k < 8; ++k) a.ps[k] += b.ps[k];
    for (int k = 0; k < 20; ++k) a.t[k] += b.t[k];
    for (int r = 0; r < 8; ++r) { a.rt[r] += b.rt[r]; for (int k = 0; k < 10; ++k) a.rp[r][k] += b.rp[r][k]; }
    for (int k = 0; k < 18; ++k) a.sx[k / 6][k % 6] += b.sx[k / 6][k % 6];
#endif
}

__device__ __forceinline__ void tally_flush(const KParams& K, const Tally& c) {
    const unsigned v[14] = {c.samples, c.traversals, c.tlas_nodes, c.tlas_leaf_indices, c.instances, c.blas_nodes,
                            c.triangles, c.materials, c.light_fetches, c.scatters, c.diffuse_scatters, c.hemi_draws, c.lit_lights, c.triangles_past_u};
    unsigned long long* g = reinterpret_cast<unsigned long long*>(K.counters);
    for (int k = 0; k < 14; ++k) {
        unsigned x = v[k];
        for (int o = 32; o > 0; o >>= 1) x += __shfl_xor(x, o);
        if ((threadIdx.x & 63) == 0 && x) atomicAdd(&g[k < 9 ? k : k + 1], (unsigned long long)x);
    }
}

#ifndef RZ_PERSIST_WAVES_PER_CU
#define RZ_PERSIST_WAVES_PER_CU 16
#endif
#ifndef RZ_GROUPS_PER_CLAIM
#define RZ_GROUPS_PER_CLAIM 8
#endif
#ifndef RZ_GROUPS_PER_CLAIM_SMALL_SPP
#define RZ_GROUPS_PER_CLAIM_SMALL_SPP 6
#endif
#define RZ_SPREAD_ON(K) (SPREAD && (K).spreadTrace != 0)
#ifndef RZ_CLAIM_RUN_SMALL_SPP
#define RZ_CLAIM_RUN_SMALL_SPP 1
#endif
#ifndef RZ_PARK_BOUNCE
#define RZ_PARK_BOUNCE 2
#endif
#ifndef RZ_DARK_UNITS
#define RZ_DARK_UNITS 1
#endif
#ifndef RZ_COMPACT_DEFAULT
#define RZ_COMPACT_DEFAULT 1
#endif
template <bool COUNT, bool GLASS, bool OVF, bool SPREAD>
__device__ __forceinline__ void render_samples_group(const KParams& K, const unsigned wblock, unsigned char* lds_raw) {
    const int lane = threadIdx.x & 63;
    const BlasStackT<OVF> bstk{reinterpret_cast<uint2*>(lds_raw) + lane,
                               OVF ? K.blasOvf + ((size_t)blockIdx.x * K.blasOvfCap) * 64 + lane : nullptr, K.blasStackCap};
    float4* addL = reinterpret_cast<float4*>(lds_raw + (size_t)K.blasStackCap * 64 * sizeof(uint2) +
                                             (size_t)K.tlasStackCap * 64 * sizeof(int));

    const int spp = K.spp;
    const int pixPerWave = spp >= 64 ? 1 : 64 / spp;
    const int nBatches = spp >= 64 ? (spp + 63) / 64 : 1;
    const int myPixInWave = spp >= 64 ? 0 : lane / spp;
    const int slot = (int)wblock * pixPerWave + myPixInWave;
    const int sumSlot = (int)wblock * pixPerWave + lane;
// ... 197 lines not shown
                        }
                        for (; k < nMine; ++k) { ch = ch + Lf[4 * k]; ch = ch + Sf[4 * k]; }
                    }
                    const float cx = __shfl(ch, 0), cy = __shfl(ch, 1), cz = __shfl(ch, 2);
                    if (sumInside) { acc.x = cx; acc.y = cy; acc.z = cz; consumed = nMine; }
                    chosen[lane] = 0;
                }
                firstPass = false;
                if (sumInside) {
                    while (consumed < nMine) {
                        const int k = firstLane + consumed;
                        int pick = -1;
#pragma unroll
                        for (int v = 0; v < 2; ++v) {
                            const int inf = vinfo[v * 64 + k];
                            if (pick < 0 && (inf & 1) && (!(inf & 2) || __float_as_uint(verL[v * 64 + k].w) == __float_as_uint(iorPix))) pick = v;
                        }
                        if (pick < 0) break;
                        const float4 L = verL[pick * 64 + k], S = verS[pick * 64 + k];
                        acc.x = acc.x + L.x; acc.y = acc.y + L.y; acc.z = acc.z + L.z;
                        acc.x = acc.x + S.x; acc.y = acc.y + S.y; acc.z = acc.z + S.z;
                        if (vinfo[pick * 64 + k] & 2) iorPix = S.w;
                        chosen[k] = pick;
                        ++consumed;
                    }
                }
                __syncthreads();
                if (rz_ballot(sumInside && consumed < nMine) == 0ull) break;
            }
            if (COUNT && mine) tally_add(c, tv[chosen[lane]]);
            __syncthreads();
        }
    }
    if (!GLASS && spp >= 64) {
        const float cx = __shfl(chan, 0), cy = __shfl(chan, 1), cz = __shfl(chan, 2);
        if (sumInside0 && lane == 0) {
            K.accum[sumPix0] = make_float4(cx, cy, cz, alpha0 + (float)spp);
            K.ior[sumPix0] = 1.0f;
        }
    } else if (sumInside) {
        acc.w += (float)spp;
        K.accum[sumPix] = acc;
        K.ior[sumPix] = iorPix;
    }
#ifdef RZ_PROF
    if (COUNT) {
        unsigned long long* pr = reinterpret_cast<unsigned long long*>(K.counters + 1);
        for (int k = 0; k < 16; ++k) if (c.p[k]) atomicAdd(&pr[k], (unsigned long long)c.p[k]);
        if (lane == 0) { atomicAdd(&pr[17], tTrace); atomicAdd(&pr[18], tAdv); atomicAdd(&pr[19], c.t[0]); atomicAdd(&pr[20], c.t[1]); atomicAdd(&pr[21], c.t[2]); for (int k = 3; k < 10; ++k) atomicAdd(&pr[19 + k], c.t[k]); }
        rz_prof_rounds(c, pr);
    }
#endif
    if (COUNT) {
        tally_flush(K, c);
        const unsigned long long pm = rz_ballot(sumInside);
        if (lane == 0 && pm) atomicAdd(&K.counters->pixels, (unsigned long long)__popcll(pm));
    }
}



struct ClaimMap {
    unsigned nGroups, perClaim, nClaims, runShift;
    __device__ __forceinline__ int group(unsigned ci, int g) const {
        const unsigned j = (unsigned)g >> runShift, w = (unsigned)g & ((1u << runShift) - 1u);
        return (int)(((j * nClaims + ci) << runShift) + w);
    }
    __device__ __forceinline__ int units_of(unsigned ci) const {
        int n = 0;
        for (unsigned g = 0; g < perClaim; ++g) n += (unsigned)group(ci, (int)g) < nGroups ? 1 : 0;
        return n;
    }
};

__device__ __forceinline__ int wmeta_load(const int* p) { return __hip_atomic_load(p, __ATOMIC_RELAXED, __HIP_MEMORY_SCOPE_AGENT); }
__device__ __forceinline__ int kth_set_lane(unsigned long long m) {
    const int lane = threadIdx.x & 63;
    int got = 0, k = 0;
    for (unsigned long long rest = m; rest != 0ull; rest &= rest - 1ull, ++k)
        if (lane == k) got = (int)__builtin_ctzll(rest);
    return got;
}

#ifndef RZ_SUM_UNROLL
#define RZ_SUM_UNROLL 8
#endif
#define RZ_ST_ADD(p, v) (*(p) = (v))
#define RZ_LD_ADD(p) (*(p))
__device__ __forceinline__ const float* zero_row(const KParams& K) { return reinterpret_cast<const float*>(K.groupCounter + 128); }
template <bool COUNT, bool GLASS>
__device__ __forceinline__ void ordered_sum_pass(const KParams& K, const bool valid, const float* __restrict__ A, const int slot, const int lane0, const unsigned lit = ~0u) {
    const int lane = threadIdx.x & 63;
    const int spp = K.spp;
    const int nBatches = (spp + 63) / 64;
    const int q = lane / 3, ch = lane - 3 * q;
    bool inside = false;
    size_t pix = 0;
    float chan = 0.0f, alpha = 0.0f;
    if (valid) {
        const int localTile = slot >> 6, l = slot & 63;
        const int tile = localTile * K.tileNRanks + K.tileRank;
        const int ty = tile / K.tilesX, tx = tile - ty * K.tilesX;
        const int px = tx * RZ_TILE_W + slot_x(l, spp < 64), py = ty * RZ_TILE_H + slot_y(l, spp < 64);
        if (slot < K.nSlots && px < K.width && py < K.height) {
            inside = true;
            pix = (size_t)py * K.width + px;
            if (K.sampleBase != 0) {
                const float4 a = K.accum[pix];
                chan = ch == 0 ? a.x : (ch == 1 ? a.y : a.z);
                alpha = a.w;
            }
        }
    }
    if (inside) {
        for (int b = 0; b < nBatches; ++b) {
            const float* Sf = A + (size_t)b * 384 + 64 * ch + lane0 + 192;
            const float* Lf = ((lit >> b) & 1u) ? Sf - 192 : zero_row(K) + lane0;
            const int cnt = spp >= 64 ? min(64, spp - b * 64) : spp;
            int k = 0;
            for (; k + RZ_SUM_UNROLL <= cnt; k += RZ_SUM_UNROLL) {
                float l[RZ_SUM_UNROLL], q8[RZ_SUM_UNROLL];
#pragma unroll
                for (int u = 0; u < RZ_SUM_UNROLL; ++u) { l[u] = RZ_LD_ADD(Lf + k + u); q8[u] = RZ_LD_ADD(Sf + k + u); }
#pragma unroll
                for (int u = 0; u < RZ_SUM_UNROLL; ++u) { chan = chan + l[u]; chan = chan + q8[u]; }
            }
            for (; k < cnt; ++k) { chan = chan + RZ_LD_ADD(Lf + k); chan = chan + RZ_LD_ADD(Sf + k); }
        }
    }
    const int l0 = q < 21 ? 3 * q : 0;
    const float cx = __shfl(chan, l0), cy = __shfl(chan, l0 + 1), cz = __shfl(chan, l0 + 2);
    if (inside && ch == 0) {
        K.accum[pix] = make_float4(cx, cy, cz, alpha + (float)spp);
        K.ior[pix] = GLASS ? A[(size_t)nBatches * 384 + lane0] : 1.0f;
    }
    if (COUNT) {
        const unsigned long long im = rz_ballot(inside && ch == 0);
        if (lane == 0 && im) atomicAdd(&K.counters->pixels, (unsigned long long)__popcll(im));
    }
}

template <bool COUNT, bool GLASS>
__device__ __forceinline__ void slot_sums(const KParams& K, const float* __restrict__ slotsBase, int* __restrict__ meta, const unsigned long long ready, int& freeCount) {
    const int lane = threadIdx.x & 63;
    const int spp = K.spp, NS = K.nWaitSlots;
    const int ppw = spp >= 64 ? 1 : 64 / spp;
    const int n = mask_count(ready);
    const int nPix = n * ppw;
    const int slotOfRank = kth_set_lane(ready);
    const int gidxOfRank = lane < n ? wmeta_load(meta + slotOfRank) : 0;
    for (int p0 = 0; p0 < nPix; p0 += 21) {
        const int q = lane / 3;
        const int p = p0 + q;
        const bool valid = q < 21 && p < nPix;
        const int r = valid ? p / ppw : 0;
        const int pin = p - r * ppw;
        const int sl = __shfl(slotOfRank, r), gidx = __shfl(gidxOfRank, r);
        ordered_sum_pass<COUNT, GLASS>(K, valid, slotsBase + (size_t)sl * K.slotFloats, gidx * ppw + pin, pin * (spp >= 64 ? 0 : spp));
    }
    if ((ready >> lane) & 1ull) meta[NS + lane] = -1;
    freeCount += n;
    __syncthreads();
}

#ifndef RZ_GLASS_BOX_MAX_DFS
#define RZ_GLASS_BOX_MAX_DFS 64
#endif
__device__ __forceinline__ bool may_hit_glass(const KParams& K, const bool cand, const v3 o, const v3 d) {
    if (K.glassBoxHint == 0 || K.nTlasDfs > RZ_GLASS_BOX_MAX_DFS || rz_ballot(cand) == 0ull) return false;
    const v3 inv = rcp3(d);
    bool hit = false;
    for (int pos = 0; pos < K.nTlasDfs; ++pos) {
        const f32x16 q = sload16(K.tlasDfs + pos);
        if (__float_as_int(q[7]) <= 0) continue;
        if ((sload1(&K.instances[__float_as_int(q[9])].flags) & 2) == 0) continue;
        float tmin;
        hit = hit || slab(o, inv, q[0], q[1], q[2], q[4], q[5], q[6], tmin);
    }
    return cand && hit;
}

__device__ __forceinline__ void rz_backstop(const KParams& K, unsigned code) {
    if ((threadIdx.x & 63) == 0) atomicOr(K.groupCounter + RZ_ERRWORD, code);
}

template <bool COUNT, bool OVF, int UNITS, bool GLASS>
__device__ __forceinline__ void render_claim_compact(const KParams& K, const ClaimMap M, const unsigned ci, const int nRedo, const int redoTop, unsigned char* lds_raw, int& wpN, int& freeCount) {
    using namespace poolf;
    const int lane = threadIdx.x & 63;
    const BlasStackT<OVF> bstk{reinterpret_cast<uint2*>(lds_raw) + lane,
                               OVF ? K.blasOvf + ((size_t)blockIdx.x * K.blasOvfCap) * 64 + lane : nullptr, K.blasStackCap};
    float* const addBase = K.wslots + (size_t)blockIdx.x * K.wslotStride;
    unsigned* const W = K.wpool + (size_t)blockIdx.x * K.wpoolStride * RZ_GPOOL_FIELDS;
    int* const meta = K.wmeta + (size_t)blockIdx.x * 4 * K.nWaitSlots;
    const int NS = K.nWaitSlots;
    const size_t WS = K.wpoolStride;
    const size_t GF = K.slotFloats;
    const int spp = K.spp;
    const int nBatches = (spp + 63) / 64;
    const bool redo = GLASS && nRedo > 0;
    const int ppw = spp >= 64 ? 1 : 64 / spp;
    const int nGroups = redo ? nRedo : M.units_of(ci);
    const int nUnits = nGroups * nBatches;
    const int pixInUnit = spp >= 64 ? 0 : lane / spp;
    const int sampInUnit = spp >= 64 ? lane : lane - pixInUnit * spp;
    auto group_of = [&](int g) -> int { return (GLASS && redo) ? wmeta_load(meta + 3 * NS + (redoTop - nRedo + g)) : M.group(ci, g); };
    int nPool = 0;
    unsigned litMask = 0u;
    int tileCached = -1, tileX = 0, tileY = 0;
    float iorCarry = 1.0f;
    Tally c = {};
    for (int unit = 0; unit < nUnits; ++unit) {
        Path P;
#ifdef RZ_PROF
        const unsigned long long tph0_ = __builtin_amdgcn_s_memtime();
#endif
        P.mode = MODE_DONE;
        P.addLight = mk3(0.0f, 0.0f, 0.0f);
        P.addSky = mk3(0.0f, 0.0f, 0.0f);
        P.usedIor = 0;
        P.ior = 1.0f;
        const int g = nBatches == 1 ? unit : unit / nBatches, b = unit - g * nBatches;
        bool mine = false;
        float iorStart = 1.0f;
        Tally cu = {};
        Tally& tu = (COUNT && GLASS) ? cu : c;
        {
            const int slot = group_of(g) * ppw + pixInUnit;
            const int localTile = slot >> 6, l = slot & 63;
            int px, py;
            if (spp >= 64 || (64 % ppw) == 0) {
                const int ut = __builtin_amdgcn_readfirstlane(localTile);
                if (ut != tileCached) {
                    tileCached = ut;
                    const int tile = ut * K.tileNRanks + K.tileRank;
                    tileY = tile / K.tilesX;
                    tileX = tile - tileY * K.tilesX;
                }
                px = tileX * RZ_TILE_W + slot_x(l, spp < 64); py = tileY * RZ_TILE_H + slot_y(l, spp < 64);
            } else {
                const int tile = localTile * K.tileNRanks + K.tileRank;
                const int ty = tile / K.tilesX, tx = tile - ty * K.tilesX;
                px = tx * RZ_TILE_W + slot_x(l, true); py = ty * RZ_TILE_H + slot_y(l, true);
            }
            const int s = b * 64 + sampInUnit;
            const bool pixInside = pixInUnit < ppw && slot < K.nSlots && px < K.width && py < K.height;
            if constexpr (GLASS) {
                iorStart = b == 0 ? ((K.sampleBase != 0 && pixInside) ? K.ior[(size_t)py * K.width + px] : 1.0f) : iorCarry;
            }
            if (pixInside && s < spp) {
                mine = true;
                const float fragx = (float)px + 0.5f, fragy = (float)py + 0.5f;
                P.uv.x = fragx / (float)K.width;
                P.uv.y = fragy / (float)K.height;
                P.fragSum = fragx + fragy;
                P.color = mk3(0.0f, 0.0f, 0.0f);
                P.samp = K.sampleBase + s;
                begin_sample<COUNT>(K, P, tu);
                if constexpr (GLASS) P.ior = iorStart;
            }
        }
        bool stopLate = !GLASS || !(COUNT || redo);
        unsigned key0 = __float_as_uint(iorStart), key1 = 0u, out0 = 0u, out1 = 0u, want = __float_as_uint(iorStart);
        int info0 = 0, info1 = 0, nextSlot = 0, chosen = 0;
        bool running = mine;
        bool resolved = false;
        float iorEnd = iorStart;
        Tally tv0 = {}, tv1 = {};
        float* const V = GLASS ? K.snap + (size_t)blockIdx.x * K.snapStride + (size_t)(RZ_SNAP_FIELDS + RZ_SNAP_TALLY) * 64 + lane : nullptr;
#ifdef RZ_PROF
        c.rnd = 0;
#endif
        for (int round = 0; round < 200; ++round) {
            if (GLASS && round == 199) rz_backstop(K, 4u);
            bool run, anyRun;
            {
                const bool late = stopLate && P.mode == MODE_SEGMENT && P.bounce >= RZ_PARK_BOUNCE;
                run = P.mode != MODE_DONE && !late;
                if constexpr (GLASS) { if (stopLate) run = run || may_hit_glass(K, late, P.o, P.d); }
                anyRun = rz_ballot(run) != 0ull;
            }
            while (anyRun) {
                if (run) {
                    HitRec h;
                    bool found = false;
#ifdef RZ_PROF
                    const unsigned long long tq0_ = __builtin_amdgcn_s_memtime();
#endif
                    int sx = 0;
                    if (!shadow_candidate<COUNT, GLASS>(P)) {
                        RZ_SITE(c, 6);
                        if constexpr (shadow_exit<COUNT, GLASS>)
                            found = trace_closest<COUNT, OVF, false, true>(K, P.o, P.d, h, bstk, tu, nullptr, shadow_exit_dist<COUNT, GLASS>(P), &sx);
                        else
                            found = trace_closest<COUNT, OVF>(K, P.o, P.d, h, bstk, tu);
                    }
#ifdef RZ_PROF
                    c.rt[c.rnd & 7] += __builtin_amdgcn_s_memtime() - tq0_;
#endif
                    advance<COUNT, GLASS, GLASS ? 1 : 0>(K, P, found, h, tu, sx);
                }
#ifdef RZ_PROF
                if (c.rnd < 7) ++c.rnd;
#endif
                const bool late = stopLate && P.mode == MODE_SEGMENT && P.bounce >= RZ_PARK_BOUNCE;
                if constexpr (GLASS) {
                    const bool ran = run;
                    run = P.mode != MODE_DONE && !late;
                    if (stopLate) run = ran && (run || may_hit_glass(K, ran && late, P.o, P.d));
                } else {
                    run = P.mode != MODE_DONE && !late;
// ... 324 lines not shown
                const unsigned bl = bestKey & 63u;
                const unsigned iorIdx = (unsigned)nBatches * 384u + (spp >= 64 ? 0u : (bl / (unsigned)spp) * (unsigned)spp);
                if (lane == 0) {
                    const size_t e = (size_t)best;
                    P.hp = mk3(__uint_as_float(LL[0 * LC + e]), __uint_as_float(LL[1 * LC + e]), __uint_as_float(LL[2 * LC + e]));
                    P.hn = mk3(__uint_as_float(LL[3 * LC + e]), __uint_as_float(LL[4 * LC + e]), __uint_as_float(LL[5 * LC + e]));
                    P.pdir = mk3(__uint_as_float(LL[6 * LC + e]), __uint_as_float(LL[7 * LC + e]), __uint_as_float(LL[8 * LC + e]));
                    P.throughput = mk3(__uint_as_float(LL[9 * LC + e]), __uint_as_float(LL[10 * LC + e]), __uint_as_float(LL[11 * LC + e]));
                    P.seed.x = __uint_as_float(LL[12 * LC + e]); P.seed.y = __uint_as_float(LL[13 * LC + e]);
                    P.samp = (int)LL[14 * LC + e]; P.bounce = (int)LL[15 * LC + e]; P.hmat = (int)LL[16 * LC + e];
                    P.color = mk3(0.0f, 0.0f, 0.0f);
                    P.ior = A[iorIdx];
                    scatter<COUNT, true, 0>(K, P, c);
                    LL[18 * LC + e] = 0xffffffffu;
                    atomicAdd(meta + 2 * NS + s, -1);
                    if (P.mode != MODE_DONE) {
                        const size_t d = (size_t)write;
                        W[OX * WS + d] = __float_as_uint(P.o.x); W[OY * WS + d] = __float_as_uint(P.o.y); W[OZ * WS + d] = __float_as_uint(P.o.z);
                        W[DX * WS + d] = __float_as_uint(P.d.x); W[DY * WS + d] = __float_as_uint(P.d.y); W[DZ * WS + d] = __float_as_uint(P.d.z);
                        W[TPX * WS + d] = __float_as_uint(P.throughput.x); W[TPY * WS + d] = __float_as_uint(P.throughput.y); W[TPZ * WS + d] = __float_as_uint(P.throughput.z);
                        W[SEEDX * WS + d] = __float_as_uint(P.seed.x); W[SEEDY * WS + d] = __float_as_uint(P.seed.y);
                        W[SAMP * WS + d] = (unsigned)P.samp;
                        W[BACK * WS + d] = (1u << 31) | ((unsigned)P.bounce << 16) | bestKey;
                        W[(size_t)(RZ_GPOOL_FIELDS - 1) * WS + d] = (unsigned)s;
                        W[IOR * WS + d] = __float_as_uint(P.ior);
                    } else {
                        A[iorIdx] = P.ior;
                        atomicAdd(meta + NS + s, -1);
                    }
                }
                write += __builtin_amdgcn_readfirstlane(P.mode != MODE_DONE ? 1 : 0);
            }
            __syncthreads();
        }
        {
            bool any = false;
            for (int e0 = 0; e0 < lateN; e0 += 64) any = any || rz_ballot(e0 + lane < lateN && LL[18 * LC + e0 + lane] != 0xffffffffu) != 0ull;
            if (!any) lateN = 0;
        }
    }
    unsigned long long ready = rz_ballot(lane < NS && wmeta_load(meta + NS + (lane < NS ? lane : 0)) == 0);
    if constexpr (GLASS) {
        const unsigned long long dirty = ready & rz_ballot(lane < NS && ((unsigned)wmeta_load(meta + 2 * NS + (lane < NS ? lane : 0)) & FULL_REDO) != 0u);
        if ((dirty >> lane) & 1ull) {
            meta[3 * NS + redoCount + __popcll(dirty & below)] = wmeta_load(meta + lane);
            meta[2 * NS + lane] = 0;
            meta[NS + lane] = -1;
        }
        redoCount += mask_count(dirty);
        RZ_GSTAT(2, mask_count(dirty));
        freeCount += mask_count(dirty);
        ready &= ~dirty;
    }
    slot_sums<COUNT, GLASS>(K, slotsBase, meta, ready, freeCount);
#ifdef RZ_PROF
    c.t[17] += __builtin_amdgcn_s_memtime() - tss0_;
#endif
    if (COUNT) {
        tally_flush(K, c);
#ifdef RZ_PROF
        unsigned long long* pr = reinterpret_cast<unsigned long long*>(K.counters + 1);
        for (int k = 0; k < 16; ++k) if (c.p[k]) atomicAdd(&pr[k], (unsigned long long)c.p[k]);
        if (lane == 0) { for (int k = 9; k < 12; ++k) atomicAdd(&pr[19 + k], c.t[k]); for (int k = 12; k < 20; ++k) atomicAdd(&pr[108 + k], c.t[k]); }
        rz_prof_rounds(c, pr);
#endif
    }
    return write;
}

template <bool COUNT, bool GLASS, bool OVF, int COMPACT>
__global__ __launch_bounds__(64, GLASS ? RZ_SAMPLES_MIN_WAVES_GLASS : RZ_SAMPLES_MIN_WAVES) void rz_render_samples(const KParams K, const unsigned nGroups, const unsigned perClaim,
                                                                                                                  const unsigned nClaims, const unsigned runShift) {
    extern __shared__ __attribute__((aligned(16))) unsigned char lds_raw[];
#ifdef RZ_PROF
    const unsigned long long wl_t0 = __builtin_amdgcn_s_memrealtime();
    unsigned wl_claims = 0;
#endif
    if constexpr (COMPACT <= 1) {
        if (perClaim == 0) {
            render_samples_group<COUNT, GLASS, OVF, COMPACT == 1>(K, blockIdx.x, lds_raw);
            return;
        }
    }
    const ClaimMap M{nGroups, perClaim, nClaims, runShift};
    if constexpr (COMPACT > 1) {
        int* const meta = K.wmeta + (size_t)blockIdx.x * 4 * K.nWaitSlots;
        if ((int)(threadIdx.x & 63) < K.nWaitSlots) meta[K.nWaitSlots + (threadIdx.x & 63)] = -1;
        __syncthreads();
        int wpN = 0, freeCount = K.nWaitSlots, redoCount = 0, lateN = 0;
        const BlasStackT<OVF> bstk{reinterpret_cast<uint2*>(lds_raw) + (threadIdx.x & 63),
                                   OVF ? K.blasOvf + ((size_t)blockIdx.x * K.blasOvfCap) * 64 + (threadIdx.x & 63) : nullptr, K.blasStackCap};
        for (unsigned long long iter = 0; iter < (1ull << 40); ++iter) {
            const bool redo = GLASS && redoCount > 0;
            unsigned ci = 0;
            int nRedo = 0;
            if (redo) {
                nRedo = redoCount < (int)perClaim ? redoCount : (int)perClaim;
            } else {
                if ((threadIdx.x & 63) == 0) ci = atomicAdd(K.groupCounter, 1u);
                ci = (unsigned)__builtin_amdgcn_readfirstlane((int)ci);
                const bool more = ci < nClaims;
                const int need = more ? M.units_of(ci) : 0;
                const int maxPasses = (K.maxBounces + 1) * (GLASS ? RZ_GLATE_CAP + 1 : 1);
                for (int guard = 0; wpN > 0 && (!more || wpN >= (int)K.wpoolChunk || freeCount < need || K.drainEachClaim != 0) && guard <= maxPasses; ++guard)
                    wpN = pool_process<COUNT, OVF, GLASS>(K, K.wpool + (size_t)blockIdx.x * K.wpoolStride * RZ_GPOOL_FIELDS, K.wpoolStride, wpN, bstk, freeCount, redoCount, lateN);
                if (wpN > 0 && (!more || freeCount < need)) rz_backstop(K, 2u);
                if (!more) {
                    if (GLASS && redoCount > 0) continue;
                    break;
                }
                if (freeCount < need) { rz_backstop(K, 1u); break; }
            }
#ifdef RZ_PROF
            ++wl_claims;
#endif
            render_claim_compact<COUNT, OVF, COMPACT, GLASS>(K, M, ci, nRedo, redoCount, lds_raw, wpN, freeCount);
            redoCount -= nRedo;
        }
    } else {
        for (;;) {
            unsigned ci = 0;
            if ((threadIdx.x & 63) == 0) ci = atomicAdd(K.groupCounter, 1u);
            ci = (unsigned)__builtin_amdgcn_readfirstlane((int)ci);
            if (ci >= nClaims) break;
#ifdef RZ_PROF
            ++wl_claims;
#endif
            const int n = M.units_of(ci);
            for (int g = 0; g < n; ++g) render_samples_group<COUNT, GLASS, OVF, COMPACT == 1>(K, (unsigned)M.group(ci, g), lds_raw);
        }
    }
#ifdef RZ_PROF
    if ((threadIdx.x & 63) == 0 && blockIdx.x < (1u << 17)) {
        rz_wave_log[blockIdx.x][0] = wl_t0;
        rz_wave_log[blockIdx.x][1] = __builtin_amdgcn_s_memrealtime();
        rz_wave_log[blockIdx.x][2] = wl_claims;
    }
#endif
}

__global__ void rz_resolve_kernel(const float4* __restrict__ accum, uchar4* __restrict__ out, int n) {
    const int i = blockIdx.x * blockDim.x + threadIdx.x;
    if (i >= n) return;
    const float4 a = accum[i];
    const float cnt = a.w > 0.0f ? a.w : 1.0f;
    const float r = clamp_(a.x / cnt, 0.0f, 1.0f), g = clamp_(a.y / cnt, 0.0f, 1.0f), b = clamp_(a.z / cnt, 0.0f, 1.0f);
    out[i] = make_uchar4((unsigned char)__builtin_rintf(r * 255.0f), (unsigned char)__builtin_rintf(g * 255.0f),
                         (unsigned char)__builtin_rintf(b * 255.0f), 255);
}

void launch_render_pixels(const KParams& K, bool counted, hipStream_t stream) {
    const int blocks = (K.nLocalTiles + WAVES_PER_BLOCK - 1) / WAVES_PER_BLOCK;
    if (blocks <= 0) return;
    const size_t perWave = (size_t)K.blasStackCap * 64 * sizeof(uint2) + (size_t)K.tlasStackCap * 64 * sizeof(int);
    const size_t lds = perWave * WAVES_PER_BLOCK;
    if (counted)
        hipLaunchKernelGGL(rz_render_pixels<true>, dim3(blocks), dim3(WAVES_PER_BLOCK * 64), lds, stream, K);
    else
        hipLaunchKernelGGL(rz_render_pixels<false>, dim3(blocks), dim3(WAVES_PER_BLOCK * 64), lds, stream, K);
}

#ifdef RZ_GSTATS
void dump_gstats() {
    unsigned long long h[8] = {};
    if (hipMemcpyFromSymbol(h, HIP_SYMBOL(rz_gstats), sizeof h) != hipSuccess) return;
    fprintf(stderr, "[rz_gstats] units %llu  resolved in the wave %llu  groups rendered again %llu  re-run rounds %llu  paths parked %llu  pooled paths that met glass %llu\n", h[0], h[1], h[2], h[3], h[4], h[5]);
    unsigned long long z[8] = {};
    (void)hipMemcpyToSymbol(HIP_SYMBOL(rz_gstats), z, sizeof z);
}
#endif
#ifdef RZ_PROF
void dump_wave_log(int nWaves) {
    static std::vector<unsigned long long> h;
    h.resize((size_t)3 * (1 << 17));
    if (hipMemcpyFromSymbol(h.data(), HIP_SYMBOL(rz_wave_log), h.size() * 8) != hipSuccess) return;
    nWaves = std::min(nWaves, 1 << 17);
    unsigned long long t0 = ~0ull, t1 = 0, sum = 0;
    std::vector<double> dur(nWaves);
    for (int i = 0; i < nWaves; ++i) {
        t0 = std::min(t0, h[3 * i]); t1 = std::max(t1, h[3 * i + 1]);
        sum += h[3 * i + 1] - h[3 * i]; dur[i] = (double)(h[3 * i + 1] - h[3 * i]) * 1e-5;
    }
    std::vector<double> sorted = dur; std::sort(sorted.begin(), sorted.end());
    double span = (double)(t1 - t0) * 1e-5;
    fprintf(stderr, "[rz_prof] waves %d  span %.2f ms  sum of lifetimes %.1f ms  avg resident waves %.0f  wave ms: min %.3f med %.3f p90 %.3f p99 %.3f max %.3f\n",
            nWaves, span, (double)sum * 1e-5, (double)sum * 1e-5 / span, sorted[0], sorted[nWaves / 2], sorted[nWaves * 9 / 10], sorted[nWaves * 99 / 100], sorted[nWaves - 1]);
    const int NS = 20; double res[NS] = {0};
    for (int i = 0; i < nWaves; ++i) {
        double a = (double)(h[3 * i] - t0) * 1e-5, b = (double)(h[3 * i + 1] - t0) * 1e-5;
        for (int s = 0; s < NS; ++s) { double lo = span * s / NS, hi = span * (s + 1) / NS; double o = std::min(b, hi) - std::max(a, lo); if (o > 0) res[s] += o / (hi - lo); }
    }
    {
        std::vector<unsigned long long> w3(nWaves);
        for (int i = 0; i < nWaves; ++i) w3[i] = h[3 * i + 2];
        std::sort(w3.begin(), w3.end());
        fprintf(stderr, "[rz_prof] third log word per wave (claims served): min %llu  p10 %llu  med %llu  p90 %llu  max %llu\n", w3[0], w3[nWaves / 10], w3[nWaves / 2], w3[nWaves * 9 / 10], w3[nWaves - 1]);
        std::vector<double> ends(nWaves);
        for (int i = 0; i < nWaves; ++i) ends[i] = (double)(h[3 * i + 1] - t0) * 1e-5;
        std::sort(ends.begin(), ends.end());
        fprintf(stderr, "[rz_prof] wave END times (ms from the first start): p1 %.3f  p10 %.3f  med %.3f  p90 %.3f  p99 %.3f  max %.3f\n", ends[nWaves / 100], ends[nWaves / 10], ends[nWaves / 2], ends[nWaves * 9 / 10], ends[nWaves * 99 / 100], ends[nWaves - 1]);
    }
    fprintf(stderr, "[rz_prof] resident waves per 5%% time slice:");
    for (int s = 0; s < NS; ++s) fprintf(stderr, " %.0f", res[s]);
    fprintf(stderr, "\n");
}
#endif

SamplesPlan plan_render_samples(int spp, int nSlots, bool glass) {
    SamplesPlan p{};
    const int pixPerWave = spp >= 64 ? 1 : 64 / spp;
    p.groups = ((long long)nSlots + pixPerWave - 1) / pixPerWave;
    static int nCU = 0;
    if (nCU == 0) {
        int dev = 0; hipDeviceProp_t prop;
        nCU = (hipGetDevice(&dev) == hipSuccess && hipGetDeviceProperties(&prop, dev) == hipSuccess && prop.multiProcessorCount > 0)
                  ? prop.multiProcessorCount : 256;
    }
    const int nBatches = (spp + 63) / 64;
    const long long units = p.groups * nBatches;
    const int claimUnits = units >= (4ll << 20) ? RZ_CLAIM_UNITS_LARGE
                         : (units >= (3ll << 18) ? RZ_GROUPS_PER_CLAIM : (spp < 64 ? RZ_GROUPS_PER_CLAIM_SMALL_SPP : std::max(1, RZ_GROUPS_PER_CLAIM / 2)));
    bool smallSppClaims = true;
    if (const char* e = std::getenv("RZ_SMALL_SPP_CLAIMS")) smallSppClaims = std::atoi(e) != 0;
    const bool persistent = (spp >= 64 || smallSppClaims) && p.groups >= (long long)nCU * RZ_PERSIST_WAVES_PER_CU * 16;
    p.perClaim = persistent ? std::max(1, claimUnits / nBatches) : 0;
    if (const char* e = std::getenv("RZ_GROUPS_PER_CLAIM")) p.perClaim = std::max(0, std::atoi(e));
    bool compact = RZ_COMPACT_DEFAULT != 0;
    if (const char* e = std::getenv("RZ_COMPACT")) compact = std::atoi(e) != 0;
    bool glassClaims = true;
    if (const char* e = std::getenv("RZ_GLASS_CLAIMS")) glassClaims = std::atoi(e) != 0;
    p.compact = compact && (!glass || glassClaims) && p.perClaim > 0 && nBatches <= RZ_CLAIM_UNITS_LARGE;
    if (spp < 64 && !p.compact) p.perClaim = 0;
    p.claimUnits = 0;
    if (p.compact) {
        p.claimUnits = (p.perClaim * nBatches > RZ_CLAIM_UNITS_SMALL) ? RZ_CLAIM_UNITS_LARGE : RZ_CLAIM_UNITS_SMALL;
        p.perClaim = std::max(1, std::min(p.perClaim, p.claimUnits / nBatches));
    }
    const long long claims = p.perClaim ? (p.groups + p.perClaim - 1) / p.perClaim : p.groups;
    p.grid = p.perClaim ? std::min<long long>(claims, (long long)nCU * RZ_PERSIST_WAVES_PER_CU) : p.groups;
    p.nClaims = p.perClaim ? claims : 0;
    p.drainEachClaim = false;
    if (const char* e = std::getenv("RZ_CROSS_CLAIM_POOL")) p.drainEachClaim = std::atoi(e) == 0;
    int run = spp >= 64 ? p.perClaim : RZ_CLAIM_RUN_SMALL_SPP;
    if (const char* e = std::getenv("RZ_CLAIM_RUN")) run = std::max(1, std::atoi(e));
    if (run > p.perClaim) run = p.perClaim;
    if (run <= 0 || (run & (run - 1)) != 0 || p.perClaim % run != 0) run = 1;
    p.runShift = 0;
    while ((1 << (p.runShift + 1)) <= run) ++p.runShift;
    return p;
}
size_t samples_lds_extra(bool glass, bool compact) {
    if (compact) return 0;
    return glass ? 4 * 64 * sizeof(float4) + 3 * 64 * sizeof(int) : 6 * 64 * sizeof(float);
}

void launch_render_samples(const KParams& K, bool counted, bool glass, hipStream_t stream) {
    const SamplesPlan plan = plan_render_samples(K.spp, K.nSlots, glass);
    const long long blocks = plan.groups, grid = plan.grid, perClaim = plan.perClaim;
    if (blocks <= 0) return;
    const bool compact = plan.compact && K.wpool != nullptr;
    const size_t lds = (size_t)K.blasStackCap * 64 * sizeof(uint2) + (size_t)K.tlasStackCap * 64 * sizeof(int) + samples_lds_extra(glass, compact);
    const dim3 g((unsigned)grid), b(64);
    const unsigned nGroups = (unsigned)blocks;
    if (perClaim && hipMemsetAsync(K.groupCounter, 0, sizeof(unsigned), stream) != hipSuccess) return;
    const bool ovf = K.blasOvfCap > 0;
#define RZ_LAUNCH_SAMPLES(C, G, O, M) hipLaunchKernelGGL((rz_render_samples<C, G, O, M>), g, b, lds, stream, K, nGroups, (unsigned)perClaim, (unsigned)plan.nClaims, (unsigned)plan.runShift)
    const bool spread = K.spreadTrace != 0 && K.spp < 64;
    if (glass && compact && plan.claimUnits == RZ_CLAIM_UNITS_LARGE) {
        if (counted) { if (ovf) RZ_LAUNCH_SAMPLES(true, true, true, RZ_CLAIM_UNITS_LARGE); else RZ_LAUNCH_SAMPLES(true, true, false, RZ_CLAIM_UNITS_LARGE); }
        else { if (ovf) RZ_LAUNCH_SAMPLES(false, true, true, RZ_CLAIM_UNITS_LARGE); else RZ_LAUNCH_SAMPLES(false, true, false, RZ_CLAIM_UNITS_LARGE); }
    } else if (glass && compact) {
        if (counted) { if (ovf) RZ_LAUNCH_SAMPLES(true, true, true, RZ_CLAIM_UNITS_SMALL); else RZ_LAUNCH_SAMPLES(true, true, false, RZ_CLAIM_UNITS_SMALL); }
        else { if (ovf) RZ_LAUNCH_SAMPLES(false, true, true, RZ_CLAIM_UNITS_SMALL); else RZ_LAUNCH_SAMPLES(false, true, false, RZ_CLAIM_UNITS_SMALL); }
    } else if (glass && spread) {
        if (counted) { if (ovf) RZ_LAUNCH_SAMPLES(true, true, true, 1); else RZ_LAUNCH_SAMPLES(true, true, false, 1); }
        else { if (ovf) RZ_LAUNCH_SAMPLES(false, true, true, 1); else RZ_LAUNCH_SAMPLES(false, true, false, 1); }
    } else if (glass) {
        if (counted) { if (ovf) RZ_LAUNCH_SAMPLES(true, true, true, 0); else RZ_LAUNCH_SAMPLES(true, true, false, 0); }
        else { if (ovf) RZ_LAUNCH_SAMPLES(false, true, true, 0); else RZ_LAUNCH_SAMPLES(false, true, false, 0); }
    } else if (compact && plan.claimUnits == RZ_CLAIM_UNITS_LARGE) {
        if (counted) { if (ovf) RZ_LAUNCH_SAMPLES(true, false, true, RZ_CLAIM_UNITS_LARGE); else RZ_LAUNCH_SAMPLES(true, false, false, RZ_CLAIM_UNITS_LARGE); }
        else { if (ovf) RZ_LAUNCH_SAMPLES(false, false, true, RZ_CLAIM_UNITS_LARGE); else RZ_LAUNCH_SAMPLES(false, false, false, RZ_CLAIM_UNITS_LARGE); }
    } else if (compact) {
        if (counted) { if (ovf) RZ_LAUNCH_SAMPLES(true, false, true, RZ_CLAIM_UNITS_SMALL); else RZ_LAUNCH_SAMPLES(true, false, false, RZ_CLAIM_UNITS_SMALL); }
        else { if (ovf) RZ_LAUNCH_SAMPLES(false, false, true, RZ_CLAIM_UNITS_SMALL); else RZ_LAUNCH_SAMPLES(false, false, false, RZ_CLAIM_UNITS_SMALL); }
    } else if (spread) {
        if (counted) { if (ovf) RZ_LAUNCH_SAMPLES(true, false, true, 1); else RZ_LAUNCH_SAMPLES(true, false, false, 1); }
        else { if (ovf) RZ_LAUNCH_SAMPLES(false, false, true, 1); else RZ_LAUNCH_SAMPLES(false, false, false, 1); }
    } else {
        if (counted) { if (ovf) RZ_LAUNCH_SAMPLES(true, false, true, 0); else RZ_LAUNCH_SAMPLES(true, false, false, 0); }
        else { if (ovf) RZ_LAUNCH_SAMPLES(false, false, true, 0); else RZ_LAUNCH_SAMPLES(false, false, false, 0); }
    }
#undef RZ_LAUNCH_SAMPLES
}

__global__ void rz_hemi0_kernel(float* out) {
    v2 z; z.x = 0.0f; z.y = 0.0f;
    const v3 d = hemisphere_local(z);
    out[0] = d.x; out[1] = d.y; out[2] = d.z;
}
int compute_hemi0(float out[3], hipStream_t stream) {
    float* d = nullptr;
    hipError_t e = hipMalloc(reinterpret_cast<void**>(&d), 3 * sizeof(float));
    if (e != hipSuccess) return -(int)e;
    hipLaunchKernelGGL(rz_hemi0_kernel, dim3(1), dim3(1), 0, stream, d);
    e = hipGetLastError();
    if (e == hipSuccess) e = hipMemcpyAsync(out, d, 3 * sizeof(float), hipMemcpyDeviceToHost, stream);
    if (e == hipSuccess) e = hipStreamSynchronize(stream);
    (void)hipFree(d);
    return e == hipSuccess ? 0 : -(int)e;
}

void launch_resolve(const float4* accum, uchar4* out, int n, hipStream_t stream) {
    hipLaunchKernelGGL(rz_resolve_kernel, dim3((n + 255) / 256), dim3(256), 0, stream, accum, out, n);
}

}
```

### rayzen_amd/csrc/hip/rz_scene_dev.h

```cpp
#pragma once
#include <stddef.h>
#include <stdint.h>

namespace rz {

struct alignas(64) DevPair {
    float lx[2], ly[2];
    float lz[2], rx[2];
    float ry[2], rz[2];
    int32_t lenc, renc;
    int32_t pad[2];
};
static_assert(sizeof(DevPair) == 64, "DevPair is one 64-B line");

struct alignas(16) DevTri {
    float v0[3]; float e1x;
    float e1y, e1z, e2x, e2y;
    float e2z; int32_t mat; int32_t src; int32_t pad;
};
static_assert(sizeof(DevTri) == 48, "DevTri is three 16-B loads");

struct alignas(16) DevTriN { float n[3]; int32_t mat; };
static_assert(sizeof(DevTriN) == 16, "DevTriN is one 16-B load");

// ... 1 lines not shown
    float inv[12];
    float fwd[12];
    float rootMin[3]; int32_t rootEnc;
    float rootMax[3]; int32_t pairBase;
    int32_t triBase;
    int32_t flags;
    int32_t pad[2];
};
static_assert(sizeof(DevInstance) == 144, "DevInstance");

struct TlasNode {
    float bmin[3]; int32_t leftFirst;
    float bmax[3]; int32_t count;
};

struct alignas(64) TlasDfs {
    float bmin[3]; int32_t first;
    float bmax[3]; int32_t count;
    int32_t skip;
    int32_t inst0;
    int32_t pad[6];
};
static_assert(sizeof(TlasDfs) == 64, "TlasDfs is one scalar fetch");
static_assert(offsetof(TlasDfs, bmin) == 0 && offsetof(TlasDfs, first) == 12 && offsetof(TlasDfs, bmax) == 16 &&
              offsetof(TlasDfs, count) == 28 && offsetof(TlasDfs, skip) == 32 && offsetof(TlasDfs, inst0) == 36 &&
              offsetof(TlasDfs, pad) == 40, "TlasDfs field offsets");

struct DevMaterial { float albedo[3], metallic, roughness, reflectivity, transparency, ior; };
struct DevLight { float posdir[4], color[3], power; };

struct DevCounters {
    unsigned long long samples, traversals, tlas_nodes, tlas_leaf_indices, instances, blas_nodes, triangles,
        materials, light_fetches, pixels, scatters, diffuse_scatters, hemi_draws, lit_lights, triangles_past_u;
};

struct KParams {
    const DevPair* pairs;
    const DevTri* tris;
    const DevInstance* instances;
    const TlasDfs* tlasDfs;
    const int32_t* tlasIndices;
    const DevMaterial* materials;
    const DevLight* lights;
    float4* accum;
    float* ior;
    DevCounters* counters;
    unsigned* groupCounter;
    int32_t nTlasDfs;
    int32_t nLights;
    int32_t nMaterials;
    int32_t width, height;
    int32_t tilesX, tilesY;
    int32_t nLocalTiles;
    int32_t tileRank, tileNRanks;
    int32_t maxBounces;
    int32_t spp, sampleBase;
    int32_t nSlots;
    int32_t blasStackCap;
    int32_t tlasStackCap;
    float invView[16];
    float invProj[16];
    float camPos[3];
    int32_t blasOvfCap;
    uint2* blasOvf;
    float* wslots;
    uint32_t wslotStride;
    const DevTriN* triN;
    float hemi0[3];
    int32_t traceRoundCap;
    int32_t spreadTrace;
    unsigned* wpool;
    uint32_t wpoolStride;
    uint32_t wpoolChunk;
    int32_t* wmeta;
    uint32_t slotFloats;
    int32_t nWaitSlots;
    int32_t claimUnits;
    int32_t glassBoxHint;
    uint32_t claimScratchFloats;
    int32_t drainEachClaim;
    int32_t regularBoxes;
    float* snap;
    uint32_t snapStride;
};

struct TlasWork {
    const float* transforms;
    DevInstance* instances;
    rz_bvh_instance* refInstances;
    TlasNode* nodes;
    int32_t* indices;
    TlasDfs* dfs;
    float* worldMin;
    float* worldMax;
    int32_t* order;
    int32_t* stack;
    int32_t* outCounts;
    int32_t* scratch;
    int n;
};

struct SamplesPlan { long long groups, grid; int perClaim; bool compact; int claimUnits; long long nClaims; int runShift; bool drainEachClaim; };

constexpr int RZ_CLAIM_UNITS_SMALL = 8, RZ_CLAIM_UNITS_LARGE = 16;
constexpr int RZ_ERRWORD = 16;
constexpr unsigned RZ_BACKSTOP_RAYS = 8u;
constexpr int RZ_POOL_FIELDS = 24;
constexpr int RZ_GPOOL_FIELDS = RZ_POOL_FIELDS + 1;
constexpr int RZ_SNAP_FIELDS = 19, RZ_SNAP_TALLY = 14;
constexpr int RZ_GLATE_FIELDS = 19, RZ_GLATE_CAP = 128;
constexpr int RZ_GVER_ROWS = 12;

}
```

### rayzen_amd/renderer.py

```python
import ctypes as C

import numpy as np

from . import _lib
from .scene import BINDING_DTYPES, BIND_INSTANCES, BIND_TLAS_INDICES, BIND_TLAS_NODES, MORPH_TRIANGLE, SKIN_TRIANGLE


class RayZenError(RuntimeError):
    def __init__(self, what, code, message):
        super().__init__(f"{what} failed ({code}): {message}")
        self.code = code


def frame_params(camera, width, height, num_lights, bounce_budget, spp, sample_base=0, tile_rank=0, tile_nranks=1):
    p = _lib.FrameParams()
    p.width, p.height = int(width), int(height)
    p.inv_view[:] = camera.inv_view.tolist()
    p.inv_proj[:] = camera.inv_proj.tolist()
    p.view[:] = camera.view.tolist()
    p.proj[:] = camera.proj.tolist()
    p.cam_pos[:] = camera.position.tolist()
    p.num_lights, p.bounce_budget = int(num_lights), int(bounce_budget)
    p.spp, p.sample_base = int(spp), int(sample_base)
    p.tile_rank, p.tile_nranks = int(tile_rank), int(tile_nranks)
# ... 217 lines not shown
        self.upload(S.BIND_INSTANCES, inst)
        self.upload(S.BIND_TLAS_NODES, tn)
        self.upload(S.BIND_TLAS_INDICES, ti)
        self.upload(S.BIND_MATERIALS, materials)
        self.upload(S.BIND_LIGHTS, lights)
        return {S.BIND_INSTANCES: inst, S.BIND_TLAS_NODES: tn, S.BIND_TLAS_INDICES: ti, S.BIND_TRIANGLES: tris}

    def read_binding(self, binding):
        need = C.c_size_t(0)
        self._check(self._L.rz_read_binding(self._c, int(binding), None, 0, C.byref(need)), "rz_read_binding")
        dt = BINDING_DTYPES[int(binding)]
        out = np.zeros(need.value // dt.itemsize, dt)
        self._check(self._L.rz_read_binding(self._c, int(binding), out.ctypes.data if out.nbytes else None, out.nbytes,
                                            C.byref(need)), "rz_read_binding")
        return out

    def set_frame(self, params):
        self._check(self._L.rz_set_frame(self._c, C.byref(params)), "rz_set_frame")
        self.width, self.height = params.width, params.height
        self._frame = _lib.FrameParams.from_buffer_copy(params)

    def set_stream(self, hip_stream):
        self._check(self._L.rz_set_stream(self._c, C.c_void_p(hip_stream)), "rz_set_stream")

    def bind_accum(self, device_ptr, nbytes):
        self._check(self._L.rz_bind_accum(self._c, C.c_void_p(device_ptr), int(nbytes)), "rz_bind_accum")

    def render(self):
        self._check(self._L.rz_render(self._c), "rz_render")

    def render_counted(self):
        cnt = _lib.Counters()
        self._check(self._L.rz_render_counted(self._c, C.byref(cnt)), "rz_render_counted")
        return {n: int(getattr(cnt, n)) for n in _lib.COUNTER_FIELDS}

    def sync(self):
        self._check(self._L.rz_sync(self._c), "rz_sync")

    def clear_accum(self):
        self._check(self._L.rz_clear_accum(self._c), "rz_clear_accum")

    def read_accum(self):
        out = np.empty((self.height, self.width, 4), np.float32)
        self._check(self._L.rz_read_accum(self._c, out.ctypes.data, out.nbytes), "rz_read_accum")
        return out

    def resolve_rgba8(self):
        out = np.empty((self.height, self.width, 4), np.uint8)
        self._check(self._L.rz_resolve_rgba8(self._c, out.ctypes.data, out.nbytes), "rz_resolve_rgba8")
        return out

    def present(self, fps=0.0, show_fps=True, show_lights=False, show_bvh=False, bvh_mode=0, selected_blas=0,
                selected_tri=0):
        p = _lib.PresentParams(float(fps), int(bool(show_fps)), int(bool(show_lights)), int(bool(show_bvh)),
                               int(bvh_mode), int(selected_blas), int(selected_tri))
        rgb = np.empty((self.height, self.width, 3), np.float32)
        rgba8 = np.empty((self.height, self.width, 4), np.uint8)
        self._check(self._L.rz_present(self._c, C.byref(p), rgba8.ctypes.data, rgba8.nbytes, rgb.ctypes.data,
                                       rgb.nbytes), "rz_present")
        return rgb, rgba8

    def last_render_ms(self):
        ms, n = C.c_float(0), C.c_int(0)
        self._check(self._L.rz_last_render_ms(self._c, C.byref(ms), C.byref(n)), "rz_last_render_ms")
        return float(ms.value), int(n.value)

    def render_history_ms(self, cap=64):
        buf = (C.c_float * cap)()
        n = self._L.rz_render_history_ms(self._c, buf, cap)
        if n < 0:
            self._check(n, "rz_render_history_ms")
        return [float(buf[k]) for k in range(n)]

    def last_kernel_name(self):
        return self._L.rz_last_kernel_name(self._c).decode()

    def debug_fail_alloc(self, nth):
        self._check(self._L.rz_debug_fail_alloc(self._c, int(nth)), "rz_debug_fail_alloc")

    def debug_last_plan(self):
        lp = _lib.LaunchPlan()
        self._check(self._L.rz_debug_last_plan(self._c, C.byref(lp)), "rz_debug_last_plan")
        return {n: int(getattr(lp, n)) for n, _ in _lib.LaunchPlan._fields_}

    def debug_read_layout(self, which):
        need = C.c_size_t(0)
        self._check(self._L.rz_debug_read_layout(self._c, int(which), None, 0, C.byref(need)), "rz_debug_read_layout")
        out = np.zeros(need.value, np.uint8)
        self._check(self._L.rz_debug_read_layout(self._c, int(which), out.ctypes.data if need.value else None, out.nbytes, C.byref(need)),
                    "rz_debug_read_layout")
        return out

    def accum_device_ptr(self):
        return self._L.rz_accum_device_ptr(self._c)

    def trace_rays(self, origins, dirs, incoherent=False):
        rays = make_rays(origins, dirs)
        hits = np.zeros(rays.shape[0], HIT_DTYPE)
        flags = _lib.RAYS_HOST | (_lib.RAYS_INCOHERENT if incoherent else 0)
        self._check(self._L.rz_trace_rays(self._c, rays.ctypes.data if rays.size else None, hits.ctypes.data if hits.size else None,
                                          rays.shape[0], flags), "rz_trace_rays")
        return {k: hits[k].copy() for k in ("t", "point", "normal", "material", "instance", "triangle", "prim")}

    def trace_rays_device(self, rays_ptr, hits_ptr, n, incoherent=False):
        self._check(self._L.rz_trace_rays(self._c, C.c_void_p(rays_ptr), C.c_void_p(hits_ptr), int(n),
                                          _lib.RAYS_INCOHERENT if incoherent else 0), "rz_trace_rays")

    def shadow_rays(self, origins, dirs, max_dist, incoherent=False):
        rays = make_rays(origins, dirs, max_dist)
        out = np.zeros(rays.shape[0], VISIBILITY_DTYPE)
        flags = _lib.RAYS_HOST | (_lib.RAYS_INCOHERENT if incoherent else 0)
        self._check(self._L.rz_shadow_rays(self._c, rays.ctypes.data if rays.size else None, out.ctypes.data if out.size else None,
                                           rays.shape[0], flags), "rz_shadow_rays")
        return out["lit"] != 0, out["visibility"].copy()

    def shadow_rays_device(self, rays_ptr, out_ptr, n, incoherent=False):
        self._check(self._L.rz_shadow_rays(self._c, C.c_void_p(rays_ptr), C.c_void_p(out_ptr), int(n),
                                           _lib.RAYS_INCOHERENT if incoherent else 0), "rz_shadow_rays")

    def pick(self, mouse_x, mouse_y, screen_w, screen_h, camera):
        o, d = pick_ray(mouse_x, mouse_y, screen_w, screen_h, camera)
        h = self.trace_rays(o[None], d[None])
        if h["instance"][0] < 0:
            return None
        return int(h["instance"][0]), int(h["triangle"][0])

    @staticmethod
    def _editor_args(camera, width, height, num_lights, ambient, clear):
        fp = frame_params(camera, width, height, 0x7fffffff if num_lights is None else num_lights, 0, 1)
        if ambient is None and clear is None:
            return fp, None
        ep = _lib.EditorParams()
        ep.ambient[:] = [0.03] * 3 if ambient is None else [float(a) for a in ambient]
        ep.clear[:] = [0.05, 0.05, 0.07, 1.0] if clear is None else [float(a) for a in clear]
        return fp, C.byref(ep)

    def render_editor(self, camera, width, height, num_lights=None, ambient=None, clear=None, rgb32f=False, hits=False,
                      incoherent=False):
        fp, ep = self._editor_args(camera, width, height, num_lights, ambient, clear)
        out8 = np.empty((height, width, 4), np.uint8)
        rgb = np.empty((height, width, 3), np.float32) if rgb32f else None
        hh = np.empty((height, width), HIT_DTYPE) if hits else None
        flags = _lib.EDITOR_HOST | (_lib.EDITOR_INCOHERENT if incoherent else 0)
        self._check(self._L.rz_render_editor(self._c, C.byref(fp), ep, out8.ctypes.data, out8.nbytes,
                                             None if rgb is None else rgb.ctypes.data, 0 if rgb is None else rgb.nbytes,
                                             None if hh is None else hh.ctypes.data, 0 if hh is None else hh.nbytes, flags),
                    "rz_render_editor")
        return out8, rgb, hh

    def render_editor_device(self, camera, width, height, rgba8_ptr=None, rgb32f_ptr=None, hits_ptr=None, num_lights=None,
                             ambient=None, clear=None, incoherent=False):
        fp, ep = self._editor_args(camera, width, height, num_lights, ambient, clear)
        n = int(width) * int(height)
        self._check(self._L.rz_render_editor(self._c, C.byref(fp), ep, C.c_void_p(rgba8_ptr), n * 4 if rgba8_ptr else 0,
                                             C.c_void_p(rgb32f_ptr), n * 12 if rgb32f_ptr else 0, C.c_void_p(hits_ptr),
                                             n * 48 if hits_ptr else 0, _lib.EDITOR_INCOHERENT if incoherent else 0),
                    "rz_render_editor")

    @staticmethod
    def _denoise_params(iterations, sigma_color, sigma_normal, sigma_plane, demodulate):
        if iterations is None and sigma_color is None and sigma_normal is None and sigma_plane is None and demodulate is None:
            return None
        p = _lib.DenoiseParams()
        p.iterations = 5 if iterations is None else int(iterations)
        p.sigma_color = 0.5 if sigma_color is None else float(sigma_color)
        p.sigma_normal = 128.0 if sigma_normal is None else float(sigma_normal)
# ... 527 lines not shown
```

Baseline: 14600 Msamples/s.

## Add sky prepass that certifies all-miss pixels and compacts the work list

Adds a prepass kernel that tests each pixel's camera ray against the TLAS and instance root boxes. Pixels whose rays miss every box have their sky contribution written directly through the ordered-sum path. Only the remaining pixels go into a compacted list that the main compact render loop claims from. This removes path-tracing work for background pixels at the cost of an extra launch, a per-pixel coarse traversal, and per-sample checks for straddling pixels.

```diff
diff --git a/include/rayzen_hip.h b/include/rayzen_hip.h
--- a/include/rayzen_hip.h
+++ b/include/rayzen_hip.h
@@ -258,6 +258,8 @@
     int32_t scratch_mib;
 } rz_launch_plan;
 int rz_debug_last_plan(rz_ctx* ctx, rz_launch_plan* out);
+
+int rz_debug_sky_prepass(rz_ctx* ctx, int64_t out[4]);
 
 typedef struct rz_ray {
     float    origin[3];
diff --git a/profiles/r08_sky_prepass/allsky_ms.py b/profiles/r08_sky_prepass/allsky_ms.py
--- /dev/null
+++ b/profiles/r08_sky_prepass/allsky_ms.py
@@ -0,0 +1,30 @@
+import os
+import sys
+
+sys.path.insert(0, os.path.dirname(os.path.dirname(os.path.dirname(os.path.abspath(__file__)))))
+from rayzen_amd import scene as S
+from rayzen_amd.renderer import Renderer, frame_params
+
+W, H, SPP, B = 1920, 1080, 64, 4
+runs = int(sys.argv[1]) if len(sys.argv) > 1 else 3
+
+
+def ms_of(sc):
+    r = Renderer(0)
+    r.upload_scene(sc)
+    r.set_frame(frame_params(sc.camera, W, H, len(sc.lights), B, SPP))
+    for _ in range(5):
+        r.render()
+    r.sync()
+    ms = r.render_history_ms()[1:]
+    r.close()
+    return min(ms)
+
+
+c2 = S.bunny_scene(n=76, aspect=W / H)
+sky = S.bunny_scene(n=76, aspect=W / H)
+sky.camera.target[:] = (0.0, 0.0, 1.0)
+sky.camera.update()
+name = os.path.basename(os.environ.get("RAYZEN_HIP_SO", "new"))
+for k in range(runs):
+    print(f"{name} run {k}: all-sky {ms_of(sky):.3f} ms   c2 {ms_of(c2):.3f} ms", flush=True)
diff --git a/profiles/r08_sky_prepass/cpu_count.py b/profiles/r08_sky_prepass/cpu_count.py
--- /dev/null
+++ b/profiles/r08_sky_prepass/cpu_count.py
@@ -0,0 +1,57 @@
+import os
+import sys
+
+import numpy as np
+
+ROOT = os.path.dirname(os.path.dirname(os.path.dirname(os.path.abspath(__file__))))
+sys.path.insert(0, ROOT)
+sys.path.insert(0, os.path.join(ROOT, "tests"))
+from oracle import rzo
+from rayzen_amd import scene as S
+from helpers import oracle_scene
+
+name = sys.argv[1] if len(sys.argv) > 1 else "c2"
+W, H = (int(sys.argv[2]), int(sys.argv[3])) if len(sys.argv) > 3 else (384, 216)
+sc = S.named_config(name)[0]
+a = sc.arrays
+cam = sc.camera
+
+
+def slab(o, d, lo, hi):
+    with np.errstate(divide="ignore", invalid="ignore"):
+        inv = 1.0 / d
+        t0, t1 = (lo - o) * inv, (hi - o) * inv
+    tmin = np.minimum(t0, t1).max(axis=1)
+    tmax = np.maximum(t0, t1).min(axis=1)
+    return tmax >= np.maximum(tmin, 0.0)
+
+
+ys, xs = np.mgrid[0:H, 0:W]
+u, v = (xs.ravel() + 0.5) / W, (ys.ravel() + 0.5) / H
+ip, iv = cam.inv_proj.astype(np.float64), cam.inv_view.astype(np.float64).reshape(4, 4).T
+cx, cy = 2.0 * u - 1.0, 2.0 * v - 1.0
+eye = np.stack([ip[0] * cx + ip[4] * cy - ip[8] + ip[12], ip[1] * cx + ip[5] * cy - ip[9] + ip[13], -np.ones_like(cx)], axis=1)
+d = eye @ iv[:3, :3].T
+d /= np.linalg.norm(d, axis=1, keepdims=True)
+o = np.broadcast_to(cam.position.astype(np.float64), d.shape)
+
+leaf = np.zeros(len(d), bool)
+for n in a[S.BIND_TLAS_NODES]:
+    if n["count"] > 0:
+        leaf |= slab(o, d, n["boundsMin"].astype(np.float64), n["boundsMax"].astype(np.float64))
+root = np.zeros(len(d), bool)
+nodes = a[S.BIND_BLAS_NODES]
+for inst in a[S.BIND_INSTANCES]:
+    r = nodes[inst["blasNodeOffset"]]
+    if r["count"] == 0 and (r["boundsMin"] > r["boundsMax"]).any():
+        continue
+    m = inst["inverseTransform"].astype(np.float64).reshape(4, 4).T
+    lo_, ld = o @ m[:3, :3].T + m[:3, 3], d @ m[:3, :3].T
+    ld /= np.linalg.norm(ld, axis=1, keepdims=True)
+    root |= slab(lo_, ld, r["boundsMin"].astype(np.float64), r["boundsMax"].astype(np.float64))
+osc = oracle_scene(sc)
+hit = np.array([rzo.trace(osc, o[k], d[k])["hit"] for k in range(len(d))])
+N = len(d)
+print(f"{name} at {W}x{H} pixel centres: hit fraction {hit.sum() / N:.3f} | enter some TLAS leaf box {leaf.sum() / N:.3f} | "
+      f"enter some instance root box {root.sum() / N:.3f} | miss every root box {1 - root.sum() / N:.3f}")
+print(f"hit pixels outside every root box: {(hit & ~root).sum()} (must be 0)")
diff --git a/rayzen_amd/_lib.py b/rayzen_amd/_lib.py
--- a/rayzen_amd/_lib.py
+++ b/rayzen_amd/_lib.py
@@ -26,6 +26,7 @@
     "rz_antialias", "rz_present_antialiased", "rz_antialias_seethrough", "rz_present_antialiased_seethrough",
     "rz_render_cost", "rz_cost_view", "rz_present_cost",
     "rz_coverage", "rz_outline",
+    "rz_debug_sky_prepass",
 )
 ABI_VERSION = 5
 HOST_SYMBOLS = (
@@ -337,7 +338,8 @@
                                 ("rz_cost_view", i, [vp, vp, vp, sz, vp, sz, vp, C.c_uint]),
                                 ("rz_present_cost", i, [vp, C.POINTER(PresentParams), vp, vp, sz, vp, sz]),
                                 ("rz_coverage", i, [vp, C.POINTER(FrameParams), vp, vp, sz, vp, sz, C.c_uint]),
-                                ("rz_outline", i, [vp, vp, vp, sz, vp, sz, vp, sz, vp, sz, C.c_uint])):
+                                ("rz_outline", i, [vp, vp, vp, sz, vp, sz, vp, sz, vp, sz, C.c_uint]),
+                                ("rz_debug_sky_prepass", i, [vp, C.POINTER(C.c_int64)])):
             try:
                 fn = getattr(L, name)
                 fn.restype, fn.argtypes = res, args
diff --git a/rayzen_amd/csrc/hip/rz_context.hip b/rayzen_amd/csrc/hip/rz_context.hip
--- a/rayzen_amd/csrc/hip/rz_context.hip
+++ b/rayzen_amd/csrc/hip/rz_context.hip
@@ -127,6 +127,10 @@
     int failAllocCountdown = 0;
     DevBuf dRawNodes, dRawIdx, dRawTris, dRelayoutWs, dClaimScratch;
     DevBuf dSnap;
+    DevBuf dSkyList;
+    bool lastSky = false;
+    long long lastSkyGroups = 0;
+    long long lastSkyPixels = 0;
     DevBuf dWavePools, dWaitMeta;
     size_t lastScratchBytes = 0;
     int* relayoutPinned = nullptr;
@@ -872,10 +876,24 @@
             K.snapStride = (uint32_t)stride;
         }
     }
+    K.skyList = nullptr; K.skyCount = nullptr;
+    if (K.wpool && !c->sceneHasTransparency && !counted && K.spp >= 64 && ensure_optional(c->dSkyList, 64 + (size_t)plan.groups * sizeof(int32_t))) {
+        K.skyCount = static_cast<unsigned*>(c->dSkyList.p);
+        K.skyList = static_cast<int32_t*>(c->dSkyList.p) + 16;
+    }
+    c->lastSky = K.nSlots > 0 && sky_prepass_on(K, plan, counted, c->sceneHasTransparency);
+    c->lastSkyGroups = c->lastSky ? plan.groups : 0;
+    c->lastSkyPixels = 0;
+    if (c->lastSky && K.tileNRanks == 1) c->lastSkyPixels = (long long)K.width * K.height;
+    else if (c->lastSky)
+        for (int lt = 0; lt < K.nLocalTiles; ++lt) {
+            const int tile = lt * K.tileNRanks + K.tileRank, ty = tile / K.tilesX, tx = tile - ty * K.tilesX;
+            c->lastSkyPixels += (long long)std::min<int>(RZ_TILE_W, K.width - tx * RZ_TILE_W) * std::min<int>(RZ_TILE_H, K.height - ty * RZ_TILE_H);
+        }
     RZ_HIP(c, hipEventRecord(c->evStart[evSlot], c->stream));
     if (K.nSlots > 0) launch_render_samples(K, counted, c->sceneHasTransparency, c->stream);
     RZ_HIP(c, hipEventRecord(c->evStop[evSlot], c->stream));
-    c->lastLaunches = K.nSlots > 0 ? 1 : 0;
+    c->lastLaunches = K.nSlots > 0 ? (c->lastSky ? 2 : 1) : 0;
     c->lastGrid = plan.grid;
     c->lastPlan = rz_launch_plan{plan.groups, plan.grid, plan.perClaim, (plan.compact && K.wpool) ? plan.claimUnits : 0,
                                  (K.spp + 63) / 64, K.spp >= 64 ? 1 : 64 / K.spp, K.blasStackCap, K.blasOvfCap,
@@ -1083,7 +1101,7 @@
     (void)hipSetDevice(c->device);
     if (c->stream) (void)hipStreamSynchronize(c->stream);
     for (DevBuf* b : {&c->dPairs, &c->dTris, &c->dInst, &c->dTlasNodes, &c->dTlasIdx, &c->dMat, &c->dLight,
-                      &c->dCounters, &c->dResolve, &c->dGroupCtr, &c->dBlasOvf, &c->ownAccum, &c->dIor, &c->dXforms, &c->dInstRef, &c->dTlasScratch, &c->dProjBoxes, &c->dBuildWs, &c->dTlasDfs, &c->dTriN, &c->dRawNodes, &c->dRawIdx, &c->dRawTris, &c->dRelayoutWs, &c->dClaimScratch, &c->dWavePools, &c->dWaitMeta, &c->dSnap,
+                      &c->dCounters, &c->dResolve, &c->dGroupCtr, &c->dBlasOvf, &c->ownAccum, &c->dIor, &c->dXforms, &c->dInstRef, &c->dTlasScratch, &c->dProjBoxes, &c->dBuildWs, &c->dTlasDfs, &c->dTriN, &c->dRawNodes, &c->dRawIdx, &c->dRawTris, &c->dRelayoutWs, &c->dClaimScratch, &c->dWavePools, &c->dWaitMeta, &c->dSnap, &c->dSkyList,
                       &c->dRayOvf, &c->dRayIn, &c->dRayOut, &c->dRayInstOff, &c->dDnGuide, &c->dDnPing, &c->dDnPong, &c->dDnOut,
                       &c->dRefitRank, &c->dRefitInstView, &c->dRefitViewOff, &c->dRefitFlags, &c->dRefitRoots,
                       &c->dTmpCol[0], &c->dTmpCol[1], &c->dTmpMom[0], &c->dTmpMom[1], &c->dTmpHits[0], &c->dTmpHits[1],
@@ -3909,6 +3927,20 @@
     return RZ_OK;
 }
 
+int rz_debug_sky_prepass(rz_ctx* c, int64_t out[4]) {
+    if (!c || !out) return fail(c, RZ_ERR_INVALID_ARG, "rz_debug_sky_prepass: null argument");
+    if (!c->timed) return fail(c, RZ_ERR_NOT_READY, "rz_debug_sky_prepass: nothing has been rendered yet");
+    out[0] = out[1] = out[2] = out[3] = 0;
+    if (!c->lastSky || !c->dSkyList.p) return RZ_OK;
+    RZ_HIP(c, hipSetDevice(c->device));
+    unsigned w[RZ_SKY_WORDS] = {};
+    RZ_HIP(c, hipMemcpyAsync(w, c->dSkyList.p, sizeof w, hipMemcpyDeviceToHost, c->stream));
+    RZ_HIP(c, hipStreamSynchronize(c->stream));
+    out[0] = (int64_t)c->lastSkyGroups;
+    out[1] = c->lastSkyPixels - (int64_t)w[0]; out[2] = (int64_t)w[0] - (int64_t)w[3]; out[3] = w[3];
+    return RZ_OK;
+}
+
 int rz_debug_fail_alloc(rz_ctx* c, int nth) {
     if (!c) return fail(nullptr, RZ_ERR_INVALID_ARG, "null context");
     c->failAllocCountdown = nth > 0 ? nth : 0;
diff --git a/rayzen_amd/csrc/hip/rz_internal.h b/rayzen_amd/csrc/hip/rz_internal.h
--- a/rayzen_amd/csrc/hip/rz_internal.h
+++ b/rayzen_amd/csrc/hip/rz_internal.h
@@ -27,6 +27,8 @@
 SamplesPlan plan_render_samples(int spp, int nSlots, bool glass);
 size_t samples_lds_extra(bool glass, bool compact);
 void launch_render_samples(const KParams& K, bool counted, bool glass, hipStream_t stream);
+bool sky_prepass_on(const KParams& K, const SamplesPlan& plan, bool counted, bool glass);
+void launch_sky_prepass(const KParams& K, hipStream_t stream);
 void launch_resolve(const float4* accum, uchar4* out, int n, hipStream_t stream);
 int compute_hemi0(float out[3], hipStream_t stream);
 #ifdef RZ_PROF
diff --git a/rayzen_amd/csrc/hip/rz_kernels.hip b/rayzen_amd/csrc/hip/rz_kernels.hip
--- a/rayzen_amd/csrc/hip/rz_kernels.hip
+++ b/rayzen_amd/csrc/hip/rz_kernels.hip
@@ -8,6 +8,7 @@
 #include "rayzen_hip.h"
 #include "rz_path.h"
 #include "rz_internal.h"
+#include "rz_ordered_sum.h"
 
 namespace rz {
 
@@ -128,8 +129,6 @@
 #ifndef RZ_SAMPLES_MIN_WAVES_GLASS
 #define RZ_SAMPLES_MIN_WAVES_GLASS 4
 #endif
-__device__ __forceinline__ int slot_x(int l, bool morton) { return morton ? ((l & 1) | ((l >> 1) & 2) | ((l >> 2) & 4)) : (l & 7); }
-__device__ __forceinline__ int slot_y(int l, bool morton) { return morton ? (((l >> 1) & 1) | ((l >> 2) & 2) | ((l >> 3) & 4)) : (l >> 3); }
 #ifdef RZ_PROF
 __device__ __forceinline__ void rz_prof_rounds(const Tally& c, unsigned long long* pr) {
     for (int k = 0; k < 8; ++k) {
@@ -493,64 +492,6 @@
     return got;
 }
 
-#ifndef RZ_SUM_UNROLL
-#define RZ_SUM_UNROLL 8
-#endif
-#define RZ_ST_ADD(p, v) (*(p) = (v))
-#define RZ_LD_ADD(p) (*(p))
-__device__ __forceinline__ const float* zero_row(const KParams& K) { return reinterpret_cast<const float*>(K.groupCounter + 128); }
-template <bool COUNT, bool GLASS>
-__device__ __forceinline__ void ordered_sum_pass(const KParams& K, const bool valid, const float* __restrict__ A, const int slot, const int lane0, const unsigned lit = ~0u) {
-    const int lane = threadIdx.x & 63;
-    const int spp = K.spp;
-    const int nBatches = (spp + 63) / 64;
-    const int q = lane / 3, ch = lane - 3 * q;
-    bool inside = false;
-    size_t pix = 0;
-    float chan = 0.0f, alpha = 0.0f;
-    if (valid) {
-        const int localTile = slot >> 6, l = slot & 63;
-        const int tile = localTile * K.tileNRanks + K.tileRank;
-        const int ty = tile / K.tilesX, tx = tile - ty * K.tilesX;
-        const int px = tx * RZ_TILE_W + slot_x(l, spp < 64), py = ty * RZ_TILE_H + slot_y(l, spp < 64);
-        if (slot < K.nSlots && px < K.width && py < K.height) {
-            inside = true;
-            pix = (size_t)py * K.width + px;
-            if (K.sampleBase != 0) {
-                const float4 a = K.accum[pix];
-                chan = ch == 0 ? a.x : (ch == 1 ? a.y : a.z);
-                alpha = a.w;
-            }
-        }
-    }
-    if (inside) {
-        for (int b = 0; b < nBatches; ++b) {
-            const float* Sf = A + (size_t)b * 384 + 64 * ch + lane0 + 192;
-            const float* Lf = ((lit >> b) & 1u) ? Sf - 192 : zero_row(K) + lane0;
-            const int cnt = spp >= 64 ? min(64, spp - b * 64) : spp;
-            int k = 0;
-            for (; k + RZ_SUM_UNROLL <= cnt; k += RZ_SUM_UNROLL) {
-                float l[RZ_SUM_UNROLL], q8[RZ_SUM_UNROLL];
-#pragma unroll
-                for (int u = 0; u < RZ_SUM_UNROLL; ++u) { l[u] = RZ_LD_ADD(Lf + k + u); q8[u] = RZ_LD_ADD(Sf + k + u); }
-#pragma unroll
-                for (int u = 0; u < RZ_SUM_UNROLL; ++u) { chan = chan + l[u]; chan = chan + q8[u]; }
-            }
-            for (; k < cnt; ++k) { chan = chan + RZ_LD_ADD(Lf + k); chan = chan + RZ_LD_ADD(Sf + k); }
-        }
-    }
-    const int l0 = q < 21 ? 3 * q : 0;
-    const float cx = __shfl(chan, l0), cy = __shfl(chan, l0 + 1), cz = __shfl(chan, l0 + 2);
-    if (inside && ch == 0) {
-        K.accum[pix] = make_float4(cx, cy, cz, alpha + (float)spp);
-        K.ior[pix] = GLASS ? A[(size_t)nBatches * 384 + lane0] : 1.0f;
-    }
-    if (COUNT) {
-        const unsigned long long im = rz_ballot(inside && ch == 0);
-        if (lane == 0 && im) atomicAdd(&K.counters->pixels, (unsigned long long)__popcll(im));
-    }
-}
-
 template <bool COUNT, bool GLASS>
 __device__ __forceinline__ void slot_sums(const KParams& K, const float* __restrict__ slotsBase, int* __restrict__ meta, const unsigned long long ready, int& freeCount) {
     const int lane = threadIdx.x & 63;
@@ -596,7 +537,8 @@
 }
 
 template <bool COUNT, bool OVF, int UNITS, bool GLASS>
-__device__ __forceinline__ void render_claim_compact(const KParams& K, const ClaimMap M, const unsigned ci, const int nRedo, const int redoTop, unsigned char* lds_raw, int& wpN, int& freeCount) {
+__device__ __forceinline__ void render_claim_compact(const KParams& K, const ClaimMap M, const unsigned ci, const int nRedo, const int redoTop, unsigned char* lds_raw, int& wpN, int& freeCount,
+                                                     const bool listed = false, const int listEntry = 0) {
     using namespace poolf;
     const int lane = threadIdx.x & 63;
     const BlasStackT<OVF> bstk{reinterpret_cast<uint2*>(lds_raw) + lane,
@@ -615,7 +557,14 @@
     const int nUnits = nGroups * nBatches;
     const int pixInUnit = spp >= 64 ? 0 : lane / spp;
     const int sampInUnit = spp >= 64 ? lane : lane - pixInUnit * spp;
-    auto group_of = [&](int g) -> int { return (GLASS && redo) ? wmeta_load(meta + 3 * NS + (redoTop - nRedo + g)) : M.group(ci, g); };
+    auto group_of = [&](int g) -> int {
+        if constexpr (!GLASS) { if (listed) return __shfl(listEntry, g); }
+        return (GLASS && redo) ? wmeta_load(meta + 3 * NS + (redoTop - nRedo + g)) : M.group(ci, g);
+    };
+    auto group_of_unit = [&](int g) -> int {
+        if constexpr (!GLASS) { if (listed) return __builtin_amdgcn_readlane(listEntry, g); }
+        return group_of(g);
+    };
     int nPool = 0;
     unsigned litMask = 0u;
     int tileCached = -1, tileX = 0, tileY = 0;
@@ -637,7 +586,7 @@
         Tally cu = {};
         Tally& tu = (COUNT && GLASS) ? cu : c;
         {
-            const int slot = group_of(g) * ppw + pixInUnit;
+            const int slot = group_of_unit(g) * ppw + pixInUnit;
             const int localTile = slot >> 6, l = slot & 63;
             int px, py;
             if (spp >= 64 || (64 % ppw) == 0) {
@@ -1128,8 +1077,17 @@
             return;
         }
     }
-    const ClaimMap M{nGroups, perClaim, nClaims, runShift};
+    ClaimMap M{nGroups, perClaim, nClaims, runShift};
     if constexpr (COMPACT > 1) {
+        bool listed = false;
+        if constexpr (!GLASS) {
+            if (K.skyList != nullptr) {
+                listed = true;
+                const unsigned n = (unsigned)__builtin_amdgcn_readfirstlane(wmeta_load(reinterpret_cast<const int*>(K.skyCount)));
+                M.nGroups = n < nGroups ? n : nGroups;
+                M.nClaims = (M.nGroups + perClaim - 1u) >> runShift;
+            }
+        }
         int* const meta = K.wmeta + (size_t)blockIdx.x * 4 * K.nWaitSlots;
         if ((int)(threadIdx.x & 63) < K.nWaitSlots) meta[K.nWaitSlots + (threadIdx.x & 63)] = -1;
         __syncthreads();
@@ -1139,13 +1097,20 @@
         for (unsigned long long iter = 0; iter < (1ull << 40); ++iter) {
             const bool redo = GLASS && redoCount > 0;
             unsigned ci = 0;
-            int nRedo = 0;
+            int nRedo = 0, listEntry = 0;
             if (redo) {
                 nRedo = redoCount < (int)perClaim ? redoCount : (int)perClaim;
             } else {
                 if ((threadIdx.x & 63) == 0) ci = atomicAdd(K.groupCounter, 1u);
                 ci = (unsigned)__builtin_amdgcn_readfirstlane((int)ci);
-                const bool more = ci < nClaims;
+                const bool more = ci < M.nClaims;
+                if constexpr (!GLASS) {
+                    if (listed && more) {
+                        const unsigned e = ci * perClaim + (threadIdx.x & 63);
+                        const unsigned v = ((threadIdx.x & 63) < perClaim && e < M.nGroups) ? (unsigned)K.skyList[e] : 0u;
+                        listEntry = (int)(v < nGroups ? v : 0u);
+                    }
+                }
                 const int need = more ? M.units_of(ci) : 0;
                 const int maxPasses = (K.maxBounces + 1) * (GLASS ? RZ_GLATE_CAP + 1 : 1);
                 for (int guard = 0; wpN > 0 && (!more || wpN >= (int)K.wpoolChunk || freeCount < need || K.drainEachClaim != 0) && guard <= maxPasses; ++guard)
@@ -1160,7 +1125,7 @@
 #ifdef RZ_PROF
             ++wl_claims;
 #endif
-            render_claim_compact<COUNT, OVF, COMPACT, GLASS>(K, M, ci, nRedo, redoCount, lds_raw, wpN, freeCount);
+            render_claim_compact<COUNT, OVF, COMPACT, GLASS>(K, M, ci, nRedo, redoCount, lds_raw, wpN, freeCount, listed, listEntry);
             redoCount -= nRedo;
         }
     } else {
@@ -1300,16 +1265,19 @@
     return glass ? 4 * 64 * sizeof(float4) + 3 * 64 * sizeof(int) : 6 * 64 * sizeof(float);
 }
 
-void launch_render_samples(const KParams& K, bool counted, bool glass, hipStream_t stream) {
-    const SamplesPlan plan = plan_render_samples(K.spp, K.nSlots, glass);
+void launch_render_samples(const KParams& Kin, bool counted, bool glass, hipStream_t stream) {
+    const SamplesPlan plan = plan_render_samples(Kin.spp, Kin.nSlots, glass);
     const long long blocks = plan.groups, grid = plan.grid, perClaim = plan.perClaim;
     if (blocks <= 0) return;
+    KParams K = Kin;
     const bool compact = plan.compact && K.wpool != nullptr;
     const size_t lds = (size_t)K.blasStackCap * 64 * sizeof(uint2) + (size_t)K.tlasStackCap * 64 * sizeof(int) + samples_lds_extra(glass, compact);
     const dim3 g((unsigned)grid), b(64);
     const unsigned nGroups = (unsigned)blocks;
     if (perClaim && hipMemsetAsync(K.groupCounter, 0, sizeof(unsigned), stream) != hipSuccess) return;
     const bool ovf = K.blasOvfCap > 0;
+    if (sky_prepass_on(K, plan, counted, glass)) launch_sky_prepass(K, stream);
+    else { K.skyList = nullptr; K.skyCount = nullptr; }
 #define RZ_LAUNCH_SAMPLES(C, G, O, M) hipLaunchKernelGGL((rz_render_samples<C, G, O, M>), g, b, lds, stream, K, nGroups, (unsigned)perClaim, (unsigned)plan.nClaims, (unsigned)plan.runShift)
     const bool spread = K.spreadTrace != 0 && K.spp < 64;
     if (glass && compact && plan.claimUnits == RZ_CLAIM_UNITS_LARGE) {
diff --git a/rayzen_amd/csrc/hip/rz_ordered_sum.h b/rayzen_amd/csrc/hip/rz_ordered_sum.h
--- /dev/null
+++ b/rayzen_amd/csrc/hip/rz_ordered_sum.h
@@ -0,0 +1,68 @@
+#pragma once
+#include <hip/hip_runtime.h>
+
+#include "rz_path.h"
+
+namespace rz {
+
+__device__ __forceinline__ int slot_x(int l, bool morton) { return morton ? ((l & 1) | ((l >> 1) & 2) | ((l >> 2) & 4)) : (l & 7); }
+__device__ __forceinline__ int slot_y(int l, bool morton) { return morton ? (((l >> 1) & 1) | ((l >> 2) & 2) | ((l >> 3) & 4)) : (l >> 3); }
+#ifndef RZ_SUM_UNROLL
+#define RZ_SUM_UNROLL 8
+#endif
+#define RZ_ST_ADD(p, v) (*(p) = (v))
+#define RZ_LD_ADD(p) (*(p))
+__device__ __forceinline__ const float* zero_row(const KParams& K) { return reinterpret_cast<const float*>(K.groupCounter + 128); }
+template <bool COUNT, bool GLASS>
+__device__ __forceinline__ void ordered_sum_pass(const KParams& K, const bool valid, const float* __restrict__ A, const int slot, const int lane0, const unsigned lit = ~0u) {
+    const int lane = threadIdx.x & 63;
+    const int spp = K.spp;
+    const int nBatches = (spp + 63) / 64;
+    const int q = lane / 3, ch = lane - 3 * q;
+    bool inside = false;
+    size_t pix = 0;
+    float chan = 0.0f, alpha = 0.0f;
+    if (valid) {
+        const int localTile = slot >> 6, l = slot & 63;
+        const int tile = localTile * K.tileNRanks + K.tileRank;
+        const int ty = tile / K.tilesX, tx = tile - ty * K.tilesX;
+        const int px = tx * RZ_TILE_W + slot_x(l, spp < 64), py = ty * RZ_TILE_H + slot_y(l, spp < 64);
+        if (slot < K.nSlots && px < K.width && py < K.height) {
+            inside = true;
+            pix = (size_t)py * K.width + px;
+            if (K.sampleBase != 0) {
+                const float4 a = K.accum[pix];
+                chan = ch == 0 ? a.x : (ch == 1 ? a.y : a.z);
+                alpha = a.w;
+            }
+        }
+    }
+    if (inside) {
+        for (int b = 0; b < nBatches; ++b) {
+            const float* Sf = A + (size_t)b * 384 + 64 * ch + lane0 + 192;
+            const float* Lf = ((lit >> b) & 1u) ? Sf - 192 : zero_row(K) + lane0;
+            const int cnt = spp >= 64 ? min(64, spp - b * 64) : spp;
+            int k = 0;
+            for (; k + RZ_SUM_UNROLL <= cnt; k += RZ_SUM_UNROLL) {
+                float l[RZ_SUM_UNROLL], q8[RZ_SUM_UNROLL];
+#pragma unroll
+                for (int u = 0; u < RZ_SUM_UNROLL; ++u) { l[u] = RZ_LD_ADD(Lf + k + u); q8[u] = RZ_LD_ADD(Sf + k + u); }
+#pragma unroll
+                for (int u = 0; u < RZ_SUM_UNROLL; ++u) { chan = chan + l[u]; chan = chan + q8[u]; }
+            }
+            for (; k < cnt; ++k) { chan = chan + RZ_LD_ADD(Lf + k); chan = chan + RZ_LD_ADD(Sf + k); }
+        }
+    }
+    const int l0 = q < 21 ? 3 * q : 0;
+    const float cx = __shfl(chan, l0), cy = __shfl(chan, l0 + 1), cz = __shfl(chan, l0 + 2);
+    if (inside && ch == 0) {
+        K.accum[pix] = make_float4(cx, cy, cz, alpha + (float)spp);
+        K.ior[pix] = GLASS ? A[(size_t)nBatches * 384 + lane0] : 1.0f;
+    }
+    if (COUNT) {
+        const unsigned long long im = rz_ballot(inside && ch == 0);
+        if (lane == 0 && im) atomicAdd(&K.counters->pixels, (unsigned long long)__popcll(im));
+    }
+}
+
+}
diff --git a/rayzen_amd/csrc/hip/rz_scene_dev.h b/rayzen_amd/csrc/hip/rz_scene_dev.h
--- a/rayzen_amd/csrc/hip/rz_scene_dev.h
+++ b/rayzen_amd/csrc/hip/rz_scene_dev.h
@@ -107,7 +107,10 @@
     int32_t regularBoxes;
     float* snap;
     uint32_t snapStride;
+    int32_t* skyList;
+    unsigned* skyCount;
 };
+constexpr int RZ_SKY_WORDS = 4;
 
 struct TlasWork {
     const float* transforms;
diff --git a/rayzen_amd/csrc/hip/rz_sky_prepass.hip b/rayzen_amd/csrc/hip/rz_sky_prepass.hip
--- /dev/null
+++ b/rayzen_amd/csrc/hip/rz_sky_prepass.hip
@@ -0,0 +1,167 @@
+#include <hip/hip_runtime.h>
+
+#include <cstdlib>
+
+#include "rayzen_hip.h"
+#include "rz_path.h"
+#include "rz_internal.h"
+#include "rz_ordered_sum.h"
+
+namespace rz {
+
+__device__ __forceinline__ bool sky_enters_any(const KParams& K, const bool live, const v3 o, const v3 d) {
+    const v3 inv = rcp3(d);
+    const int nDfs = K.nTlasDfs;
+    int idx = live ? 0 : nDfs;
+    bool enters = false;
+    int pos = 0;
+    for (int step = 0; pos < nDfs && step < nDfs; ++step) {
+        const f32x16 q = sload16(K.tlasDfs + pos);
+        const bool at = idx == pos;
+        float tmin;
+        const bool box = slab(o, inv, q[0], q[1], q[2], q[4], q[5], q[6], tmin);
+        const bool pass = at & box & !(tmin > 1e30f);
+        const int count = __float_as_int(q[7]), skip = __float_as_int(q[8]);
+        if (count > 0) {
+            if (rz_ballot(pass) != 0ull) {
+                const int first = __float_as_int(q[3]);
+                for (int i = 0; i < count; ++i) {
+                    const int instIdx = i == 0 ? __float_as_int(q[9]) : sload1(K.tlasIndices + first + i);
+                    const DevInstance* __restrict__ I = K.instances + instIdx;
+                    f32x8 m0, r0;
+                    f32x4s m1, r1;
+                    sload12(I->inv, m0, m1);
+                    sload12(I->rootMin, r0, r1);
+                    const float mi[12] = {m0[0], m0[1], m0[2], m0[3], m0[4], m0[5], m0[6], m0[7], m1[0], m1[1], m1[2], m1[3]};
+                    const v3 lo = x34_point(mi, o);
+                    const v3 ld = normalize(x34_dir(mi, d));
+                    const v3 linv = rcp3(ld);
+                    float tminRoot;
+                    bool go = slab(lo, linv, r0[0], r0[1], r0[2], r0[4], r0[5], r0[6], tminRoot);
+                    go = go && !(tminRoot > 1e30f) && !(__float_as_int(r1[1]) & 1);
+                    enters = enters || (pass && go);
+                }
+            }
+            if (at) idx = skip;
+            pos = skip;
+        } else if (count < 0) {
+            if (at) idx = pass ? pos + 1 : skip;
+            pos = rz_ballot(pass) != 0ull ? pos + 1 : skip;
+        } else {
+            if (at) idx = skip;
+            pos = skip;
+        }
+    }
+    return enters;
+}
+
+#ifndef RZ_SKY_TILES_PER_WAVE
+#define RZ_SKY_TILES_PER_WAVE 4
+#endif
+__global__ __launch_bounds__(64) void rz_sky_prepass(const KParams K, const int pairs) {
+    extern __shared__ __attribute__((aligned(16))) float sky_rows[];
+    const int lane = threadIdx.x & 63;
+    const int spp = K.spp;
+    const int nBatches = (spp + 63) / 64;
+    const int perPass = min(2 * pairs, 21);
+    const int tile0 = blockIdx.x * RZ_SKY_TILES_PER_WAVE;
+    unsigned maskLo = 0u, maskHi = 0u;
+    unsigned nStraddlers = 0u, nListed = 0u;
+  for (int t = 0; t < RZ_SKY_TILES_PER_WAVE; ++t) {
+    const int localTile = tile0 + t;
+    if (localTile >= K.nLocalTiles) break;
+    const int tile = localTile * K.tileNRanks + K.tileRank;
+    const int ty = tile / K.tilesX, tx = tile - ty * K.tilesX;
+    const v3 cam = mk3(K.camPos[0], K.camPos[1], K.camPos[2]);
+
+    const int px = tx * RZ_TILE_W + slot_x(lane, false), py = ty * RZ_TILE_H + slot_y(lane, false);
+    const bool inside = localTile * 64 + lane < K.nSlots && px < K.width && py < K.height;
+    v2 uvc;
+    uvc.x = ((float)px + 0.5f) / (float)K.width;
+    uvc.y = ((float)py + 0.5f) / (float)K.height;
+    const bool coarse = sky_enters_any(K, inside, cam, camera_ray_centre(K.invProj, K.invView, uvc));
+    const unsigned long long listedA = rz_ballot(inside && coarse);
+    unsigned long long listedB = 0ull;
+
+    int nInPass = 0;
+    int myPix = 0;
+    auto rows_of = [&](int j) -> float* { return sky_rows + 192 + (size_t)(j >> 1) * nBatches * 384 - ((j & 1) ? 192 : 0); };
+    auto flush = [&]() {
+        __syncthreads();
+        const int q = lane / 3;
+        const bool valid = q < 21 && q < nInPass;
+        ordered_sum_pass<false, false>(K, valid, rows_of(valid ? q : 0), localTile * 64 + myPix, 0, 0u);
+        __syncthreads();
+        nInPass = 0;
+    };
+    for (unsigned long long rest = rz_ballot(inside && !coarse); rest != 0ull; rest &= rest - 1ull) {
+        const int k = (int)__builtin_ctzll(rest);
+        const int kx = tx * RZ_TILE_W + slot_x(k, false), ky = ty * RZ_TILE_H + slot_y(k, false);
+        float* const A = rows_of(nInPass);
+        bool sky = true;
+        for (int b = 0; b < nBatches && sky; ++b) {
+            const int s = b * 64 + lane;
+            const bool mine = s < spp;
+            Path P;
+            Tally c = {};
+            const float fragx = (float)kx + 0.5f, fragy = (float)ky + 0.5f;
+            P.uv.x = fragx / (float)K.width;
+            P.uv.y = fragy / (float)K.height;
+            P.fragSum = fragx + fragy;
+            P.samp = K.sampleBase + s;
+            begin_sample<false>(K, P, c);
+            if (rz_ballot(sky_enters_any(K, mine, P.o, P.d)) != 0ull) { sky = false; break; }
+            const float t = 0.5f * (normalize(P.d).y + 1.0f);
+            const v3 skyc = mk3(mix_(0.15f, 0.5f, t), mix_(0.25f, 0.7f, t), mix_(0.45f, 1.0f, t));
+            const v3 addSky = mine ? P.throughput * skyc : mk3(0.0f, 0.0f, 0.0f);
+            float* const S = A + (size_t)b * 384 + 192;
+            S[lane] = addSky.x; S[64 + lane] = addSky.y; S[128 + lane] = addSky.z;
+        }
+        if (!sky) { listedB |= 1ull << k; continue; }
+        if (lane / 3 == nInPass) myPix = k;
+        if (++nInPass == perPass) flush();
+    }
+    if (nInPass > 0) flush();
+
+    const unsigned long long listed = listedA | listedB;
+    if (lane == t) { maskLo = (unsigned)listed; maskHi = (unsigned)(listed >> 32); }
+    nListed += (unsigned)__popcll(listed);
+    nStraddlers += (unsigned)__popcll(listedB);
+  }
+    if (nListed != 0u) {
+        unsigned base = 0;
+        if (lane == 0) base = atomicAdd(K.skyCount, nListed);
+        base = (unsigned)__builtin_amdgcn_readfirstlane((int)base);
+        for (int t = 0; t < RZ_SKY_TILES_PER_WAVE; ++t) {
+            const unsigned long long m = ((unsigned long long)(unsigned)__builtin_amdgcn_readlane((int)maskHi, t) << 32) |
+                                         (unsigned)__builtin_amdgcn_readlane((int)maskLo, t);
+            const unsigned at = base + (unsigned)__popcll(m & ((1ull << lane) - 1ull));
+            if (((m >> lane) & 1ull) && at < (unsigned)K.nSlots) K.skyList[at] = (tile0 + t) * 64 + lane;
+            base += (unsigned)__popcll(m);
+        }
+    }
+    if (lane == 0 && nStraddlers != 0u) atomicAdd(K.skyCount + 3, nStraddlers);
+}
+
+#ifndef RZ_SKY_PREPASS_DEFAULT
+#define RZ_SKY_PREPASS_DEFAULT 1
+#endif
+bool sky_prepass_on(const KParams& K, const SamplesPlan& plan, bool counted, bool glass) {
+    bool on = RZ_SKY_PREPASS_DEFAULT != 0;
+    if (const char* e = std::getenv("RZ_SKY_PREPASS")) on = std::atoi(e) != 0;
+    return on && !glass && !counted && plan.compact && K.wpool != nullptr && K.spp >= 64 && plan.perClaim > 0 &&
+           (1 << plan.runShift) == plan.perClaim && K.skyList != nullptr && K.skyCount != nullptr;
+}
+
+static int sky_pairs(int nBatches) { return (int)std::max<size_t>(1, std::min<size_t>(11, (10240 - 768) / ((size_t)nBatches * 1536))); }
+
+void launch_sky_prepass(const KParams& K, hipStream_t stream) {
+    if (K.nLocalTiles <= 0) return;
+    if (hipMemsetAsync(K.skyCount, 0, RZ_SKY_WORDS * sizeof(unsigned), stream) != hipSuccess) return;
+    const int pairs = sky_pairs((K.spp + 63) / 64);
+    const size_t lds = (192 + (size_t)pairs * ((K.spp + 63) / 64) * 384) * sizeof(float);
+    const unsigned grid = (unsigned)((K.nLocalTiles + RZ_SKY_TILES_PER_WAVE - 1) / RZ_SKY_TILES_PER_WAVE);
+    hipLaunchKernelGGL(rz_sky_prepass, dim3(grid), dim3(64), lds, stream, K, pairs);
+}
+
+}
diff --git a/rayzen_amd/renderer.py b/rayzen_amd/renderer.py
--- a/rayzen_amd/renderer.py
+++ b/rayzen_amd/renderer.py
@@ -323,6 +323,11 @@
         lp = _lib.LaunchPlan()
         self._check(self._L.rz_debug_last_plan(self._c, C.byref(lp)), "rz_debug_last_plan")
         return {n: int(getattr(lp, n)) for n, _ in _lib.LaunchPlan._fields_}
+
+    def debug_sky_prepass(self):
+        out = (C.c_int64 * 4)()
+        self._check(self._L.rz_debug_sky_prepass(self._c, out), "rz_debug_sky_prepass")
+        return dict(groups=int(out[0]), certified=int(out[1]), listed_coarse=int(out[2]), listed_exact=int(out[3]))
 
     def debug_read_layout(self, which):
         need = C.c_size_t(0)
```

New measurement: 13920 Msamples/s. 4.6% lower.
